# Eclectic-Sheep/sheeprl

Measured on NVIDIA H100. Metric: Dreamer-V3 train-steps/sec (S, bs16 seq64 horizon15, 64x64x3 obs), higher is better.
Workload: dtype f32

## Files before the change

include/b200rl.h:

```cpp
#ifndef B200RL_H_
#define B200RL_H_

#include <cuda_runtime_api.h>

#ifdef __cplusplus
extern "C" {
#endif

const char* b200rl_last_error(void);
int b200rl_abi_version(void);
const char* b200rl_build_arch(void);
int b200rl_device_check(void);

int b200rl_gemm_f32(const float* A, const float* B, float* C, const float* bias, int M, int N, int K, int lda, int ldb,
                    int ldc, int transA, int transB, int accumulate, cudaStream_t stream);
int b200rl_set_matmul_precision(int tf32_passes);
int b200rl_get_matmul_precision(void);
int b200rl_gemm_tc_supported(const float* A, const float* B, int M, int N, int K, int lda, int ldb, int transA,
                             int transB);
int b200rl_gemm_tc(const float* A, const float* B, float* C, const float* bias, int M, int N, int K, int lda, int ldb,
                   int ldc, int transA, int transB, int accumulate, cudaStream_t stream);
int b200rl_gemm_ln_supported(const float* A, const float* W, int M, int N, int K, int lda, int ldw, int mode);
int b200rl_gemm_ln(const float* A, const float* W, int M, int N, int K, int lda, int ldw, const float* gamma,
                   const float* beta, float eps, int act, float* pre, long long ldpre, float* out, long long ldout,
                   int mode, const float* h_prev, long long ldh, float* h_out, long long ldho, float* h_out2,
                   long long ldho2, cudaStream_t stream);
int b200rl_ln_act_fwd(const float* X, const float* gamma, const float* beta, float* Y, long long M, int C,
                      long long ldx, long long ldy, float eps, int act, cudaStream_t stream);
int b200rl_ln_act_bwd(const float* X, const float* gamma, const float* beta, const float* dY, float* dX, float* dgamma,
                      float* dbeta, long long M, int C, long long ldx, long long lddy, long long lddx, float eps,
                      int act, int accumulate, cudaStream_t stream);
int b200rl_col_sum(const float* X, float* out, long long M, int C, long long ldx, int accumulate, cudaStream_t stream);

int b200rl_obs_prep(const void* obs_nchw, int is_uint8, float* out_nhwc, long long NB, int C, int HW,
                    cudaStream_t stream);
int b200rl_transpose_batched(const float* X, float* Y, int NB, int a, int b, cudaStream_t stream);
int b200rl_transpose2d(const float* X, float* Y, int rows, int cols, long long ldx, long long ldy, cudaStream_t stream);
int b200rl_conv_down(const float* big, const float* W, float* small_, int NB, int h, int w, int Cs, int Cb,
                     cudaStream_t stream);
int b200rl_conv_up(const float* small_, const float* W, float* big, const float* bias, int NB, int h, int w, int Cs,
                   int Cb, cudaStream_t stream);
int b200rl_conv_wgrad(const float* small_, const float* big, float* dW, int NB, int h, int w, int Cs, int Cb,
                      int accumulate, cudaStream_t stream);
int b200rl_thin_down_supported(int w, int Cs, int Cb);
int b200rl_thin_up_supported(int Cs, int Cb);
int b200rl_thin_wgrad_supported(int Cs, int Cb);
int b200rl_conv_wgrad_tc_supported(int NB, int h, int w, int Cs, int Cb);
long long b200rl_conv_wgrad_tc_workspace(int NB, int h, int w, int Cs, int Cb);
int b200rl_conv_wgrad_tc(const float* small_, const float* big, float* dW, float* workspace, int NB, int h, int w,
                         int Cs, int Cb, int accumulate, cudaStream_t stream);
int b200rl_conv_tc_supported(int mode_up, int NB, int h, int w, int Cs, int Cb);
long long b200rl_conv_pack_floats(int mode_up, int Cs, int Cb);
int b200rl_conv_pack(const float* W, float* Wpacked, int mode_up, int Cs, int Cb, cudaStream_t stream);
int b200rl_conv_down_tc(const float* big, const float* Wpacked, float* small_, int NB, int h, int w, int Cs, int Cb,
                        cudaStream_t stream);
int b200rl_conv_up_tc(const float* small_, const float* Wpacked, float* big, const float* bias, int NB, int h, int w,
                      int Cs, int Cb, cudaStream_t stream);

int b200rl_gru_gate_fwd(const float* G, const float* Hin, float* Hout, long long M, int R, long long ldg,
                        long long ldhi, long long ldho, cudaStream_t stream);
int b200rl_gru_gate_bwd(const float* G, const float* Hin, const float* dH, float* dG, float* dHin, long long M, int R,
                        long long ldg, long long ldhi, long long lddh, long long lddg, long long lddhi,
                        cudaStream_t stream);
int b200rl_mask_mix(const float* prev, const float* init_row, const float* first, float* out, long long M, int C,
                    long long ldp, long long ldo, cudaStream_t stream);
int b200rl_mask_bwd(const float* dIn, const float* first, float* dPrev, float* dInit, int M, int C, long long ldi,
                    long long ldp, cudaStream_t stream);
int b200rl_cat_sample(const float* raw, const float* noise, float* onehot, float* mix_out, long long M, int groups,
                      int classes, long long ldr, long long ldn, long long ldo, long long ldm, float unimix,
                      cudaStream_t stream);
int b200rl_head_sample_supported(const float* X, const float* W, int Kin, int A, long long ldx, long long ldw);
int b200rl_head_sample(const float* X, const float* W, const float* bias, const float* noise, float* raw, float* onehot,
                       long long M, int Kin, int A, long long ldx, long long ldw, long long ldr, long long ldn,
                       long long ldo, float unimix, cudaStream_t stream);
int b200rl_cat_sample_bwd(const float* raw, const float* dz, const float* dmix, float* draw, long long M, int groups,
                          int classes, long long ldr, long long lddz, long long lddm, long long lddr, float unimix,
                          cudaStream_t stream);
int b200rl_kl_loss_grad(const float* post_mix, const float* prior_mix, float* d_post, float* d_prior, float* rows,
                        long long M, int groups, int classes, long long ldp, long long ldq, long long lddp,
                        long long lddq, float kl_dyn, float kl_rep, float free_nats, float regularizer, float scale,
                        cudaStream_t stream);
typedef struct b200rl_rssm_scan_args {
  int T, B, S, D, R, A, Dx, Dt, Dr, ld_lat, ld_wr1;
  float eps, unimix;
  const float *W_in, *lnx_g, *lnx_b, *W_g, *lng_g, *lng_b, *W_t1, *lnt_g, *lnt_b, *W_t2, *b_t2;
  const float *W_r1, *lnr_g, *lnr_b, *W_r2, *b_r2;
  const float *h0, *z0;
  const float *pe, *actions, *first, *noise;
  float* latent;
  float *z_in, *h_in, *a_in, *x_pre, *x_act, *g_pre, *g_ln, *tr_pre, *tr_act, *rp_pre, *rp_act;
  float *post_raw, *prior_raw, *post_mix, *prior_mix;
  void* workspace;
  long long workspace_bytes;
} b200rl_rssm_scan_args;
typedef struct b200rl_rssm_scan_grads {
  const float *d_latent, *d_post_mix, *d_prior_mix;
  float *d_post_raw, *d_prior_raw, *d_rp_act, *d_rp_pre, *d_tr_act, *d_tr_pre, *d_g_ln, *d_g_pre, *d_x_act, *d_x_pre;
  float* d_h0;
  const float *q_r, *q_g, *q_x;
} b200rl_rssm_scan_grads;
long long b200rl_rssm_scan_workspace_bytes(int T, int B, int S, int D, int Dx, int R, int Dr);
int b200rl_rssm_scan_fwd(const b200rl_rssm_scan_args* args, cudaStream_t stream);
int b200rl_rssm_scan_bwd(const b200rl_rssm_scan_args* args, const b200rl_rssm_scan_grads* grads, cudaStream_t stream);
int b200rl_rssm_scan_check(const b200rl_rssm_scan_args* args, int backward);
int b200rl_rssm_scan_error(const void* workspace, cudaStream_t stream);
int b200rl_rssm_scan_profile(const void* workspace, long long* out64, cudaStream_t stream);

int b200rl_mse_loss_grad(const float* pred, const float* target, float* loss_row, float* grad, long long M, int P,
                         float scale, cudaStream_t stream);
int b200rl_twohot_loss_grad(const float* logits, const float* x, const float* weight, float* loss_row, float* dlogits,
                            long long M, int nbins, long long ldl, long long ldd, float low, float high, float scale,
                            int accumulate, cudaStream_t stream);
int b200rl_bce_loss_grad(const float* logit, const float* target, float* loss_row, float* dlogit, long long M,
                         float loss_scale, float scale, cudaStream_t stream);
int b200rl_twohot_mean(const float* logits, float* out, long long M, int nbins, long long ldl, float low, float high,
                       cudaStream_t stream);
int b200rl_lambda_returns(const float* rew, const float* val, const float* cont_logit, const float* true_cont,
                          float* lam, float* discount, int H, int N, float gamma, float lmbda, cudaStream_t stream);
int b200rl_moments_update(const float* x, long long n, float* state_low_high, float* out_offset_invscale, float decay,
                          float max_, float p_low, float p_high, cudaStream_t stream);
int b200rl_actor_loss_grad(const float* raw, const float* actions, const float* lam, const float* val,
                           const float* discount, const float* moments, float* rows, float* draw, long long M,
                           const int* head_dims_host, int n_heads, float unimix, float ent_coef, float scale,
                           cudaStream_t stream);
int b200rl_sum_rows(const float* X, float* out, long long M, int C, long long ldx, float scale, cudaStream_t stream);
int b200rl_weighted_mean(const float* x, const float* w, float* out, long long n, float scale, cudaStream_t stream);

int b200rl_sumsq(const float* x, long long n, double* out, cudaStream_t stream);
int b200rl_adam_step(float* p, const float* g, float* m, float* v, const double* normsq, const int* step_dev,
                     float* norm_out, long long n, float max_norm, float lr, float b1, float b2, float eps,
                     cudaStream_t stream);
int b200rl_adam_step_wd(float* p, const float* g, float* m, float* v, const double* normsq, const int* step_dev,
                        float* norm_out, long long n, float max_norm, float lr, float b1, float b2, float eps,
                        float weight_decay, cudaStream_t stream);
int b200rl_rmsprop_step(float* p, const float* g, float* square_avg, float* momentum_buf, float* grad_avg,
                        const double* normsq, float* norm_out, long long n, float max_norm, float lr, float alpha,
                        float eps, float weight_decay, float momentum, cudaStream_t stream);
int b200rl_ema(float* target, const float* src, long long n, float tau, cudaStream_t stream);
int b200rl_fill_exponential(float* out, long long n, unsigned long long seed, unsigned int stream_id,
                            const int* counter_dev, cudaStream_t stream);
int b200rl_zero(float* x, long long n, cudaStream_t stream);
int b200rl_copy2d(const float* src, float* dst, long long M, int C, long long lds, long long ldd, cudaStream_t stream);
int b200rl_axpy(const float* x, float* y, long long n, float alpha, cudaStream_t stream);
int b200rl_affine(const float* x, float* y, long long n, float alpha, float beta, cudaStream_t stream);
int b200rl_symlog(const float* x, float* y, long long M, int C, long long ldx, long long ldy, cudaStream_t stream);
int b200rl_tanh_fwd(const float* x, float* y, long long n, cudaStream_t stream);
int b200rl_tanh_bwd(const float* y, const float* dy, float* dx, long long n, int accumulate, cudaStream_t stream);
int b200rl_increment(int* p, cudaStream_t stream);

int b200rl_replay_gather(const void* storage, const long long* idx, void* out, int n_samples, int batch, int seq_len,
                         long long row_bytes, cudaStream_t stream);
int b200rl_replay_scatter(const void* src, const long long* dst_rows, void* storage, long long n_rows,
                          long long row_bytes, cudaStream_t stream);
int b200rl_gae(const float* rewards, const float* values, const float* dones, const float* next_value, float* returns,
               float* advantages, int T, int E, float gamma, float lmbda, cudaStream_t stream);

int b200rl_bgemm(const float* A, long long sam, long long sak, long long strideA, const float* B, long long sbk,
                 long long sbn, long long strideB, float* C, long long ldc, long long strideC, const float* bias,
                 long long strideBias, const float* aux, long long ldaux, long long strideAux, float* rsum,
                 long long strideRsum, int M, int N, int K, int nets, int epilogue, int accumulate, cudaStream_t stream);
int b200rl_sac_sample_fwd(const float* head, const float* eps, const float* scale, const float* abias, float* action,
                          long long ld_action, float* logp, float* tanh_out, int B, int A, cudaStream_t stream);
int b200rl_sac_sample_bwd(const float* head, const float* eps, const float* tanh_y, const float* scale,
                          const float* dact, long long stride_net, int nets, const float* log_alpha, float* dhead, int B,
                          int A, cudaStream_t stream);
int b200rl_sac_target(const float* q_target, long long stride_net, int nets, const float* logp, const float* rewards,
                      const float* terminated, const float* log_alpha, float gamma, float* y, int B, cudaStream_t stream);
int b200rl_sac_critic_loss(const float* q, long long stride_net, int nets, const float* y, float* dq, float* loss_out,
                           int B, cudaStream_t stream);
int b200rl_sac_actor_loss(const float* q, long long stride_net, int nets, const float* logp, const float* log_alpha,
                          float target_entropy, float* dq, float* actor_loss, float* alpha_loss, float* dlog_alpha, int B,
                          cudaStream_t stream);
int b200rl_fill_normal(float* out, long long n, unsigned long long seed, unsigned int stream_id, const int* counter_dev,
                       cudaStream_t stream);

int b200rl_droq_actor_loss(const float* q, long long stride_net, int nets, const float* logp, const float* log_alpha,
                           float target_entropy, float* dq, float* actor_loss, float* alpha_loss, float* dlog_alpha,
                           int B, cudaStream_t stream);
int b200rl_dropout_mask(unsigned int* mask, long long n_words, float p, unsigned long long seed, unsigned int stream_id,
                        const int* counter_dev, cudaStream_t stream);
int b200rl_dropout_ln_relu_supported(int H);
int b200rl_dropout_ln_relu_fwd(const float* z, const unsigned int* mask, float p, const float* gamma, const float* beta,
                               long long stride_param, float eps, float* y, float* stats, int nets, int B, int H,
                               cudaStream_t stream);
int b200rl_dropout_ln_relu_bwd(const float* dy, const float* y, const float* z, const unsigned int* mask, float p,
                               const float* stats, const float* gamma, long long stride_param, float* dz, float* dgamma,
                               float* dbeta, int nets, int B, int H, cudaStream_t stream);

int b200rl_im2col(const float* x, float* col, int B, int H, int W, int C, int k, int stride, cudaStream_t stream);
int b200rl_col2im(const float* dcol, const float* act, float* dx, int B, int H, int W, int C, int k, int stride,
                  cudaStream_t stream);
int b200rl_ppo_loss(const float* head, const float* actions, const float* old_logp, const float* adv,
                    const float* values, const float* old_values, const float* returns, float* dhead, float* dvalues,
                    float* losses, int B, const int* head_dims, int n_heads, int is_continuous, int clip_vloss,
                    int normalize_adv, float clip_coef, float vf_coef, float ent_coef, cudaStream_t stream);

int b200rl_ppo_loss_masked(const float* head, const float* actions, const float* old_logp, const float* adv,
                           const float* values, const float* old_values, const float* returns, const float* mask,
                           float* dhead, float* dvalues, float* losses, int B, const int* head_dims, int n_heads,
                           int is_continuous, int clip_vloss, int normalize_adv, float clip_coef, float vf_coef,
                           float ent_coef, cudaStream_t stream);
int b200rl_a2c_loss(const float* head, const float* actions, const float* adv, const float* values, const float* returns,
                    float* dhead, float* dvalues, float* losses, int N, int seg, const int* head_dims, int n_heads,
                    int is_continuous, int normalize_adv, int reduce_sum, float vf_coef, float ent_coef,
                    cudaStream_t stream);
int b200rl_lstm_seq_fwd(const float* xw, const float* W_hh, const float* h0, const float* c0, const int* lengths,
                        float* out, float* gates, float* cs, float* hT, float* cT, int T, int B, int H,
                        cudaStream_t stream);
int b200rl_lstm_seq_bwd(const float* d_out, const float* W_hh, const float* gates, const float* cs, const float* c0,
                        const int* lengths, float* d_gates, int T, int B, int H, cudaStream_t stream);

int b200rl_onehot_linear_supported(int S, int K, int A, int N);
int b200rl_onehot_linear(const float* z, const float* act, const float* WT, float* out, long long M, int S, int K, int A,
                         int N, long long ldz, long long lda, long long ldo, cudaStream_t stream);
int b200rl_onehot_linear_ln_supported(const float* WT, const float* gamma, const float* beta, const float* out,
                                      const float* pre, int N, long long ldo, long long ldpre);
int b200rl_onehot_linear_ln(const float* z, const float* act, const float* WT, const float* gamma, const float* beta,
                            float eps, float* pre, long long ldpre, float* out, long long M, int S, int K, int A, int N,
                            long long ldz, long long lda, long long ldo, cudaStream_t stream);

int b200rl_cont_action_fwd(const float* head, const float* eps, float* action, long long lda, float* ent, long long M,
                           int A, float min_std, float max_std, float init_std, float clip, cudaStream_t stream);
int b200rl_cont_action_bwd(const float* head, const float* eps, const float* d_action, long long ldd,
                           const float* discount, float* dhead, long long M, int A, float min_std, float max_std,
                           float init_std, float clip, float ent_scale, cudaStream_t stream);
int b200rl_lambda_returns_bwd(const float* cont_logit, const float* discount, const float* moments, const float* lam,
                              const float* val, const float* ent, float* d_val, float* d_rew, float* rows, int H, int N,
                              float gamma, float lmbda, float ent_coef, float scale, cudaStream_t stream);
int b200rl_twohot_mean_bwd(const float* logits, const float* d_mean, float* d_logits, long long M, int nb, long long ldl,
                           long long ldd, float low, float high, cudaStream_t stream);

int b200rl_conv_wgrad_mn_supported(int NB, int h, int w, int Cs, int Cb);
int b200rl_conv_wgrad_mn(const float* small_, const float* big, float* G, int NB, int h, int w, int Cs, int Cb,
                         cudaStream_t stream);

int b200rl_ppo_act(const float* head, const float* noise, float* actions, float* logp, int B, const int* head_dims,
                   int n_heads, int is_continuous, int greedy, cudaStream_t stream);

#ifdef __cplusplus
}
#endif
#endif
```

sheeprl_b200/csrc/gemm_tc.cu:

```cuda
#include <cuda.h>
#include <cudaTypedefs.h>

#include <mutex>
#include <unordered_map>

#include "common.cuh"

namespace {

constexpr int BM = 128, BK = 32;
constexpr int NTHREADS = 384;
constexpr int NSPLIT_THREADS = 96;
constexpr int NCONS_WARPS = 8;
constexpr int PRODUCER_REGS = 56, CONSUMER_REGS = 224;
template <int BN> constexpr int stages_for() { return BN == 128 ? 3 : 5; }

__device__ __forceinline__ uint32_t smem_u32(const void* p) { return (uint32_t)__cvta_generic_to_shared(p); }

__device__ __forceinline__ void mbar_init(uint64_t* bar, uint32_t count) {
  asm volatile("mbarrier.init.shared::cta.b64 [%0], %1;" ::"r"(smem_u32(bar)), "r"(count) : "memory");
}
__device__ __forceinline__ void mbar_expect_tx(uint64_t* bar, uint32_t bytes) {
  asm volatile("mbarrier.arrive.expect_tx.shared::cta.b64 _, [%0], %1;" ::"r"(smem_u32(bar)), "r"(bytes) : "memory");
}
__device__ __forceinline__ void mbar_arrive(uint64_t* bar) {
  asm volatile("mbarrier.arrive.shared::cta.b64 _, [%0];" ::"r"(smem_u32(bar)) : "memory");
}
__device__ __forceinline__ bool mbar_try_wait(uint64_t* bar, uint32_t parity) {
  uint32_t ok;
  asm volatile(
      "{\n\t"
      ".reg .pred p;\n\t"
      "mbarrier.try_wait.parity.shared::cta.b64 p, [%1], %2;\n\t"
      "selp.u32 %0, 1, 0, p;\n\t"
      "}"
      : "=r"(ok)
      : "r"(smem_u32(bar)), "r"(parity)
      : "memory");
  return ok != 0;
}
__device__ __forceinline__ void mbar_wait(uint64_t* bar, uint32_t parity) {
  if (mbar_try_wait(bar, parity)) return;
  const long long t0 = clock64();
  while (!mbar_try_wait(bar, parity)) {
    if (clock64() - t0 > 2000000000LL) asm volatile("trap;");
  }
}
__device__ __forceinline__ bool elect_one() {
  uint32_t pred;
  asm volatile(
      "{\n\t"
      ".reg .pred p;\n\t"
      "elect.sync _|p, 0xffffffff;\n\t"
      "selp.u32 %0, 1, 0, p;\n\t"
      "}"
      : "=r"(pred));
  return pred != 0;
}
__device__ __forceinline__ void tma_load_2d(void* smem_dst, const CUtensorMap* map, uint64_t* bar, int c0, int c1) {
  asm volatile(
      "cp.async.bulk.tensor.2d.shared::cluster.global.mbarrier::complete_tx::bytes [%0], [%1, {%3, %4}], [%2];" ::"r"(
          smem_u32(smem_dst)),
      "l"(map), "r"(smem_u32(bar)), "r"(c0), "r"(c1)
      : "memory");
}
__device__ __forceinline__ void tma_load_4d(void* smem_dst, const CUtensorMap* map, uint64_t* bar, int c0, int c1, int c2,
                                            int c3) {
  asm volatile(
      "cp.async.bulk.tensor.4d.shared::cluster.global.mbarrier::complete_tx::bytes [%0], [%1, {%3, %4, %5, %6}], [%2];" ::"r"(
          smem_u32(smem_dst)),
      "l"(map), "r"(smem_u32(bar)), "r"(c0), "r"(c1), "r"(c2), "r"(c3)
      : "memory");
}

__device__ __forceinline__ void wgmma_tf32(float (&d)[32], const uint32_t (&a)[4], uint64_t desc_b, int scale_d) {
  asm volatile(
      "{\n\t.reg .pred p;\n\tsetp.ne.b32 p, %37, 0;\n\twgmma.mma_async.sync.aligned.m64n64k8.f32.tf32.tf32 {%0, %1, %2, %3, %4, %5, %6, %7, %8, %9, %10, %11, %12, %13, %14, %15, %16, %17, %18, %19, %20, %21, %22, %23, %24, %25, %26, %27, %28, %29, %30, %31}, {%32, %33, %34, %35}, %36, p, 1, 1;\n\t}"
      : "+f"(d[0]), "+f"(d[1]), "+f"(d[2]), "+f"(d[3]), "+f"(d[4]), "+f"(d[5]), "+f"(d[6]), "+f"(d[7]), "+f"(d[8]), "+f"(d[9]), "+f"(d[10]), "+f"(d[11]), "+f"(d[12]), "+f"(d[13]), "+f"(d[14]), "+f"(d[15]), "+f"(d[16]), "+f"(d[17]), "+f"(d[18]), "+f"(d[19]), "+f"(d[20]), "+f"(d[21]), "+f"(d[22]), "+f"(d[23]), "+f"(d[24]), "+f"(d[25]), "+f"(d[26]), "+f"(d[27]), "+f"(d[28]), "+f"(d[29]), "+f"(d[30]), "+f"(d[31])
      : "r"(a[0]), "r"(a[1]), "r"(a[2]), "r"(a[3]), "l"(desc_b), "r"(scale_d));
}
__device__ __forceinline__ void wgmma_tf32(float (&d)[64], const uint32_t (&a)[4], uint64_t desc_b, int scale_d) {
  asm volatile(
      "{\n\t.reg .pred p;\n\tsetp.ne.b32 p, %69, 0;\n\twgmma.mma_async.sync.aligned.m64n128k8.f32.tf32.tf32 {%0, %1, %2, %3, %4, %5, %6, %7, %8, %9, %10, %11, %12, %13, %14, %15, %16, %17, %18, %19, %20, %21, %22, %23, %24, %25, %26, %27, %28, %29, %30, %31, %32, %33, %34, %35, %36, %37, %38, %39, %40, %41, %42, %43, %44, %45, %46, %47, %48, %49, %50, %51, %52, %53, %54, %55, %56, %57, %58, %59, %60, %61, %62, %63}, {%64, %65, %66, %67}, %68, p, 1, 1;\n\t}"
      : "+f"(d[0]), "+f"(d[1]), "+f"(d[2]), "+f"(d[3]), "+f"(d[4]), "+f"(d[5]), "+f"(d[6]), "+f"(d[7]), "+f"(d[8]), "+f"(d[9]), "+f"(d[10]), "+f"(d[11]), "+f"(d[12]), "+f"(d[13]), "+f"(d[14]), "+f"(d[15]), "+f"(d[16]), "+f"(d[17]), "+f"(d[18]), "+f"(d[19]), "+f"(d[20]), "+f"(d[21]), "+f"(d[22]), "+f"(d[23]), "+f"(d[24]), "+f"(d[25]), "+f"(d[26]), "+f"(d[27]), "+f"(d[28]), "+f"(d[29]), "+f"(d[30]), "+f"(d[31]), "+f"(d[32]), "+f"(d[33]), "+f"(d[34]), "+f"(d[35]), "+f"(d[36]), "+f"(d[37]), "+f"(d[38]), "+f"(d[39]), "+f"(d[40]), "+f"(d[41]), "+f"(d[42]), "+f"(d[43]), "+f"(d[44]), "+f"(d[45]), "+f"(d[46]), "+f"(d[47]), "+f"(d[48]), "+f"(d[49]), "+f"(d[50]), "+f"(d[51]), "+f"(d[52]), "+f"(d[53]), "+f"(d[54]), "+f"(d[55]), "+f"(d[56]), "+f"(d[57]), "+f"(d[58]), "+f"(d[59]), "+f"(d[60]), "+f"(d[61]), "+f"(d[62]), "+f"(d[63])
      : "r"(a[0]), "r"(a[1]), "r"(a[2]), "r"(a[3]), "l"(desc_b), "r"(scale_d));
}
__device__ __forceinline__ void wgmma_fence() { asm volatile("wgmma.fence.sync.aligned;" ::: "memory"); }
__device__ __forceinline__ void wgmma_commit() { asm volatile("wgmma.commit_group.sync.aligned;" ::: "memory"); }
__device__ __forceinline__ void wgmma_wait_all() { asm volatile("wgmma.wait_group.sync.aligned 0;" ::: "memory"); }
template <int N>
__device__ __forceinline__ void fence_regs(float (&r)[N]) {
#pragma unroll
  for (int i = 0; i < N; ++i) asm volatile("" : "+f"(r[i])::"memory");
}
template <int N, int W>
__device__ __forceinline__ void fence_regs(uint32_t (&r)[N][W]) {
#pragma unroll
  for (int i = 0; i < N; ++i)
#pragma unroll
    for (int j = 0; j < W; ++j) asm volatile("" : "+r"(r[i][j])::"memory");
}

__device__ __forceinline__ uint64_t make_desc(uint32_t smem_addr) {
  uint64_t d = 0;
  d |= (uint64_t)((smem_addr & 0x3FFFF) >> 4);
  d |= (uint64_t)1 << 16;
  d |= (uint64_t)(1024 >> 4) << 32;
  d |= (uint64_t)1 << 62;
  return d;
}

__device__ __forceinline__ uint32_t kmajor_off(int r, int k) {
  return (uint32_t)(r * 128 + ((((k >> 2) ^ r) & 7) << 4) + (k & 3) * 4);
}
__device__ __forceinline__ uint32_t mnmajor_off(int r, int k) {
  return (uint32_t)((r >> 5) * 4096 + k * 128 + (((((r & 31) >> 2) ^ k) & 7) << 4) + (r & 3) * 4);
}

template <int BN>
struct Smem {
  static constexpr int STAGES = stages_for<BN>();
  float a[STAGES][BM * BK];
  float b[STAGES][BN * BK];
  float b_hi[STAGES][BN * BK];
  float b_lo[STAGES][BN * BK];
  uint64_t full[STAGES], split[STAGES], empty[STAGES];
};

constexpr int CH = 4;

constexpr int MODE_GEMM = 0, MODE_DOWN = 1, MODE_UP = 2;
constexpr int MODE_UP4 = 3;
constexpr int GROUP_M = 16;
struct TileGeo {
  int mode;
  int h, w, NB;
  int bw, bh, bn;
  int tiles_x, tiles_y;
  int chunks;
  int Cout;
  int ksplits;
  float* part;
  int mpad, ldw;
  int force_part;
  int passes;
  int a_mn, b_mn;
  int mtiles;
  int ntiles;
  int wg;
};

template <int BN, int PASSES>
__global__ void __launch_bounds__(NTHREADS, 1)
gemm_tc_kernel(const __grid_constant__ CUtensorMap mapA, const __grid_constant__ CUtensorMap mapB, float* __restrict__ C,
               const float* __restrict__ bias, int M, int N, int K, int ldc, int accumulate, const TileGeo geo) {
  constexpr int STAGES = Smem<BN>::STAGES;
  extern __shared__ __align__(1024) unsigned char smem_raw[];
  Smem<BN>& s = *reinterpret_cast<Smem<BN>*>(smem_raw + ((1024u - (smem_u32(smem_raw) & 1023u)) & 1023u));
  const int warp = threadIdx.x >> 5, lane = threadIdx.x & 31;
  const int mtiles = geo.mtiles * geo.ntiles, tstride = gridDim.y;
  auto tile_mn = [&](int id, int& tm, int& tn) {
    if (geo.ntiles == 1) { tm = id; tn = 0; return; }
    const int per = GROUP_M * geo.ntiles, grp = id / per, first = grp * GROUP_M;
    const int gsz = min(GROUP_M, geo.mtiles - first), r = id - grp * per;
    tn = r / gsz;
    tm = first + (r - tn * gsz);
  };
  int kb_base = 0, nkb = (K + BK - 1) / BK;
  if (geo.mode == MODE_GEMM && geo.ksplits > 1) {
    const int per = (nkb + geo.ksplits - 1) / geo.ksplits;
    kb_base = (int)blockIdx.z * per;
    nkb = min(per, nkb - kb_base);
  }
  const int py = (int)blockIdx.z >> 1, px = (int)blockIdx.z & 1;
  auto tile_origin = [&](int id, int& tx0, int& ty0, int& tn0) {
    tx0 = (id % geo.tiles_x) * geo.bw;
    ty0 = ((id / geo.tiles_x) % geo.tiles_y) * geo.bh;
    tn0 = (id / (geo.tiles_x * geo.tiles_y)) * geo.bn;
  };

  if (threadIdx.x == 0) {
    for (int i = 0; i < STAGES; ++i) {
      mbar_init(&s.full[i], 1);
      mbar_init(&s.split[i], NSPLIT_THREADS / 32);
      mbar_init(&s.empty[i], NCONS_WARPS);
    }
    asm volatile("fence.mbarrier_init.release.cluster;" ::: "memory");
  }
  __syncthreads();

  if (warp < 4) {
    asm volatile("setmaxnreg.dec.sync.aligned.u32 %0;" ::"n"(PRODUCER_REGS));
    if (warp == 0) {
      const bool leader = elect_one();
      int it = 0;
      for (int tile = blockIdx.y; tile < mtiles; tile += tstride) {
        int tm, tn;
        tile_mn(tile, tm, tn);
        const int m0 = tm * BM, n0 = tn * BN;
        int tx0 = 0, ty0 = 0, tn0 = 0;
        if (geo.mode != MODE_GEMM) tile_origin(tm, tx0, ty0, tn0);
        for (int kb = 0; kb < nkb; ++kb, ++it) {
          const int st = it % STAGES;
          if (it >= STAGES) mbar_wait(&s.empty[st], ((it / STAGES) - 1) & 1);
          if (leader) {
            mbar_expect_tx(&s.full[st], (uint32_t)((BM + BN) * BK * sizeof(float)));
            if (geo.mode == MODE_GEMM) {
              const int k0 = (kb_base + kb) * BK;
              if (geo.wg) {
                const int x0 = k0 % geo.w, y0 = (k0 / geo.w) % geo.h, i0 = k0 / (geo.w * geo.h);
                for (int j = 0; j < BM / 32; ++j) {
                  const int r0 = m0 + 32 * j, tap = r0 / geo.Cout, ch = r0 - tap * geo.Cout;
                  tma_load_4d(s.a[st] + j * 1024, &mapA, &s.full[st], ch, 2 * x0 - 1 + (tap & 3), 2 * y0 - 1 + (tap >> 2), i0);
                }
              } else if (!geo.a_mn) tma_load_2d(s.a[st], &mapA, &s.full[st], k0, m0);
              else
                for (int j = 0; j < BM / 32; ++j) tma_load_2d(s.a[st] + j * 1024, &mapA, &s.full[st], m0 + 32 * j, k0);
              if (!geo.b_mn) tma_load_2d(s.b[st], &mapB, &s.full[st], k0, n0);
              else
                for (int j = 0; j < BN / 32; ++j) tma_load_2d(s.b[st] + j * 1024, &mapB, &s.full[st], n0 + 32 * j, k0);
            } else {
              const int tap = kb / geo.chunks, ch = (kb - tap * geo.chunks) * BK;
              int x, y;
              if (geo.mode == MODE_DOWN)     { x = 2 * tx0 - 1 + (tap & 3); y = 2 * ty0 - 1 + (tap >> 2); }
              else if (geo.mode == MODE_UP4) { x = tx0 + (tap % 3) - 1;     y = ty0 + (tap / 3) - 1; }
              else                           { x = tx0 + px - (tap & 1);    y = ty0 + py - (tap >> 1); }
              tma_load_4d(s.a[st], &mapA, &s.full[st], ch, x, y, tn0);
              tma_load_2d(s.b[st], &mapB, &s.full[st], kb * BK, n0 + (geo.mode == MODE_UP ? (int)blockIdx.z * geo.Cout : 0));
            }
          }
          __syncwarp();
        }
      }
    } else {
      const int t = threadIdx.x - 32;
      int ntl = 0;
      for (int tile = blockIdx.y; tile < mtiles; tile += tstride) ++ntl;
      const int total_kb = ntl * nkb;
      const bool b_mn = geo.b_mn != 0;
      for (int kb = 0; kb < total_kb; ++kb) {
        const int st = kb % STAGES;
        mbar_wait(&s.full[st], (kb / STAGES) & 1);
        const char* raw = reinterpret_cast<const char*>(s.b[st]);
        char* bh = reinterpret_cast<char*>(s.b_hi[st]);
        char* bl = reinterpret_cast<char*>(s.b_lo[st]);
#pragma unroll 4
        for (int w = t; w < BN * BK / 4; w += NSPLIT_THREADS) {
          int n, kc;
          float4 v;
          if (!b_mn) {
            n = w >> 3; kc = w & 7;
            v = *reinterpret_cast<const float4*>(raw + kmajor_off(n, 4 * kc));
          } else {
            n = w % BN; kc = w / BN;
            v.x = *reinterpret_cast<const float*>(raw + mnmajor_off(n, 4 * kc));
            v.y = *reinterpret_cast<const float*>(raw + mnmajor_off(n, 4 * kc + 1));
            v.z = *reinterpret_cast<const float*>(raw + mnmajor_off(n, 4 * kc + 2));
            v.w = *reinterpret_cast<const float*>(raw + mnmajor_off(n, 4 * kc + 3));
          }
          float4 h;
          h.x = __uint_as_float(__float_as_uint(v.x) & 0xffffe000u);
          h.y = __uint_as_float(__float_as_uint(v.y) & 0xffffe000u);
          h.z = __uint_as_float(__float_as_uint(v.z) & 0xffffe000u);
          h.w = __uint_as_float(__float_as_uint(v.w) & 0xffffe000u);
          const uint32_t o = kmajor_off(n, 4 * kc);
          *reinterpret_cast<float4*>(bh + o) = h;
          if (PASSES == 3) *reinterpret_cast<float4*>(bl + o) = make_float4(v.x - h.x, v.y - h.y, v.z - h.z, v.w - h.w);
        }
        asm volatile("fence.proxy.async.shared::cta;" ::: "memory");
        __syncwarp();
        if (lane == 0) mbar_arrive(&s.split[st]);
      }
    }
  } else {
    asm volatile("setmaxnreg.inc.sync.aligned.u32 %0;" ::"n"(CONSUMER_REGS));
    constexpr int NACC = BN / 2;
    const int cw = (warp >> 2) - 1, wq = warp & 3, g = lane >> 2, tq = lane & 3;
    const int r0 = cw * 64 + wq * 16 + g;
    const bool a_mn_tile = geo.a_mn != 0;
    const uint64_t dbh_base = make_desc(smem_u32(s.b_hi[0])), dbl_base = make_desc(smem_u32(s.b_lo[0]));
    constexpr uint64_t STAGE_STEP = (uint64_t)(BN * BK * sizeof(float)) >> 4;
    int it = 0;
    for (int tile = blockIdx.y; tile < mtiles; tile += tstride) {
      int tm, tn;
      tile_mn(tile, tm, tn);
      const int m0 = tm * BM, n0 = tn * BN;
      int tx0 = 0, ty0 = 0, tn0 = 0;
      if (geo.mode != MODE_GEMM) tile_origin(tm, tx0, ty0, tn0);
      float acc[NACC], cacc[NACC];
#pragma unroll
      for (int j = 0; j < NACC; ++j) { acc[j] = 0.f; cacc[j] = 0.f; }
      for (int kb = 0; kb < nkb; ++kb, ++it) {
        const int st = it % STAGES;
        const uint32_t ph = (it / STAGES) & 1;
        mbar_wait(&s.full[st], ph);
        mbar_wait(&s.split[st], ph);
        const char* araw = reinterpret_cast<const char*>(s.a[st]);
        uint32_t ahi[4][4], alo[4][4];
#pragma unroll
        for (int ks = 0; ks < 4; ++ks)
#pragma unroll
          for (int e = 0; e < 4; ++e) {
            const int r = r0 + 8 * (e & 1), k = 8 * ks + tq + 4 * (e >> 1);
            const uint32_t x = *reinterpret_cast<const uint32_t*>(araw + (a_mn_tile ? mnmajor_off(r, k) : kmajor_off(r, k)));
            ahi[ks][e] = x & 0xffffe000u;
            if (PASSES == 3) alo[ks][e] = __float_as_uint(__uint_as_float(x) - __uint_as_float(x & 0xffffe000u));
          }
        const bool chunk_start = (kb % CH) == 0;
        const uint64_t dbh0 = dbh_base + (uint64_t)st * STAGE_STEP, dbl0 = dbl_base + (uint64_t)st * STAGE_STEP;
        fence_regs(cacc);
        fence_regs(ahi);
        if (PASSES == 3) fence_regs(alo);
        wgmma_fence();
#pragma unroll
        for (int ks = 0; ks < 4; ++ks) {
          const uint64_t ob = (uint64_t)ks * 2;
          const int keep = !(chunk_start && ks == 0);
          if (PASSES == 3) {
            wgmma_tf32(cacc, ahi[ks], dbl0 + ob, keep);
            wgmma_tf32(cacc, alo[ks], dbh0 + ob, 1);
            wgmma_tf32(cacc, ahi[ks], dbh0 + ob, 1);
          } else {
            wgmma_tf32(cacc, ahi[ks], dbh0 + ob, keep);
          }
        }
        wgmma_commit();
        wgmma_wait_all();
        fence_regs(cacc);
        fence_regs(ahi);
        if (PASSES == 3) fence_regs(alo);
        __syncwarp();
        if (lane == 0) mbar_arrive(&s.empty[st]);
        if ((kb % CH) == CH - 1 || kb == nkb - 1) {
#pragma unroll
          for (int j = 0; j < NACC; ++j) acc[j] += cacc[j];
        }
      }
#pragma unroll
      for (int hh = 0; hh < 2; ++hh) {
        const int r = r0 + 8 * hh;
        const int row = m0 + r;
        bool row_ok = row < M;
        size_t row_off = (size_t)row * ldc;
        int wi = 0, hi = 0, ni = 0;
        if (geo.mode != MODE_GEMM) {
          wi = r % geo.bw; hi = (r / geo.bw) % geo.bh; ni = r / (geo.bw * geo.bh);
          const int n = tn0 + ni, y = ty0 + hi, x = tx0 + wi;
          row_ok = n < geo.NB;
          if (geo.mode == MODE_DOWN) row_off = (((size_t)n * geo.h + y) * geo.w + x) * (size_t)ldc;
          else row_off = (((size_t)n * (2 * geo.h) + (2 * y + py)) * (2 * geo.w) + (2 * x + px)) * (size_t)ldc;
        }
        if (geo.mode == MODE_UP4) {
          if (!row_ok) continue;
          const size_t n = (size_t)(tn0 + ni);
          const int y = ty0 + hi, x = tx0 + wi;
#pragma unroll
          for (int j = 0; j < NACC / 4; ++j) {
            const int c = 8 * j + 2 * tq, p = c >> 5, ch = c & 31;
            float* dst = C + ((n * (2 * geo.h) + (2 * y + (p >> 1))) * (2 * geo.w) + (2 * x + (p & 1))) * (size_t)32 + ch;
            float2 o = make_float2(acc[4 * j + 2 * hh], acc[4 * j + 2 * hh + 1]);
            if (bias) { o.x += bias[ch]; o.y += bias[ch + 1]; }
            *reinterpret_cast<float2*>(dst) = o;
          }
          continue;
        }
        if (geo.mode == MODE_GEMM && (geo.ksplits > 1 || geo.force_part)) {
          float* prow = geo.part + ((size_t)blockIdx.z * geo.mpad + (size_t)row) * geo.ldw + n0;
#pragma unroll
          for (int j = 0; j < NACC / 4; ++j)
            *reinterpret_cast<float2*>(prow + 8 * j + 2 * tq) = make_float2(acc[4 * j + 2 * hh], acc[4 * j + 2 * hh + 1]);
          continue;
        }
        if (!row_ok) continue;
        float* crow = C + row_off;
#pragma unroll
        for (int j = 0; j < NACC / 4; ++j) {
          const int cb = n0 + 8 * j + 2 * tq;
          float v0 = acc[4 * j + 2 * hh], v1 = acc[4 * j + 2 * hh + 1];
          if (cb + 1 < N && ((reinterpret_cast<uintptr_t>(crow + cb) & 7) == 0)) {
            if (bias) { v0 += bias[cb]; v1 += bias[cb + 1]; }
            if (accumulate) { const float2 q = *reinterpret_cast<const float2*>(crow + cb); v0 += q.x; v1 += q.y; }
            *reinterpret_cast<float2*>(crow + cb) = make_float2(v0, v1);
          } else {
            if (cb < N) crow[cb] = v0 + (bias ? bias[cb] : 0.f) + (accumulate ? crow[cb] : 0.f);
            if (cb + 1 < N) crow[cb + 1] = v1 + (bias ? bias[cb + 1] : 0.f) + (accumulate ? crow[cb + 1] : 0.f);
          }
        }
      }
    }
  }
}

struct MapKey {
  const void* ptr; int rows, cols, ld, box_rows;
  bool operator==(const MapKey& o) const { return ptr == o.ptr && rows == o.rows && cols == o.cols && ld == o.ld && box_rows == o.box_rows; }
};
struct MapHash {
  size_t operator()(const MapKey& k) const {
    size_t h = std::hash<const void*>()(k.ptr);
    h ^= std::hash<long long>()(((long long)k.rows << 32) ^ k.cols) + 0x9e3779b97f4a7c15ull + (h << 6) + (h >> 2);
    h ^= std::hash<long long>()(((long long)k.ld << 8) ^ k.box_rows) + 0x9e3779b97f4a7c15ull + (h << 6) + (h >> 2);
    return h;
  }
};
std::unordered_map<MapKey, CUtensorMap, MapHash> g_maps;
std::mutex g_maps_mu;

typedef CUresult (*EncodeTiledFn)(CUtensorMap*, CUtensorMapDataType, cuuint32_t, void*, const cuuint64_t*, const cuuint64_t*,
                                  const cuuint32_t*, const cuuint32_t*, CUtensorMapInterleave, CUtensorMapSwizzle,
                                  CUtensorMapL2promotion, CUtensorMapFloatOOBfill);
EncodeTiledFn encode_tiled() {
  static EncodeTiledFn fn = nullptr;
  if (!fn) {
    void* p = nullptr;
    cudaDriverEntryPointQueryResult q;
    if (cudaGetDriverEntryPoint("cuTensorMapEncodeTiled", &p, cudaEnableDefault, &q) == cudaSuccess &&
        q == cudaDriverEntryPointSuccess)
      fn = reinterpret_cast<EncodeTiledFn>(p);
  }
  return fn;
}

int get_map(const float* ptr, int rows, int cols, int ld, int box_rows, CUtensorMap* out) {
  MapKey key{ptr, rows, cols, ld, box_rows};
  std::lock_guard<std::mutex> lk(g_maps_mu);
  auto it = g_maps.find(key);
  if (it != g_maps.end()) { *out = it->second; return B200RL_OK; }
  CUtensorMap m;
  cuuint64_t dims[2] = {(cuuint64_t)cols, (cuuint64_t)rows};
  cuuint64_t strides[1] = {(cuuint64_t)ld * sizeof(float)};
  cuuint32_t box[2] = {(cuuint32_t)BK, (cuuint32_t)box_rows};
  cuuint32_t estr[2] = {1, 1};
  EncodeTiledFn enc = encode_tiled();
  if (!enc) { b200rl_set_error("cuTensorMapEncodeTiled is not available from this driver"); return B200RL_ERR_CUDA; }
  CUresult r = enc(&m, CU_TENSOR_MAP_DATA_TYPE_FLOAT32, 2, const_cast<float*>(ptr), dims, strides, box,
                                      estr, CU_TENSOR_MAP_INTERLEAVE_NONE,
                                      CU_TENSOR_MAP_SWIZZLE_128B,
                                      CU_TENSOR_MAP_L2_PROMOTION_L2_256B, CU_TENSOR_MAP_FLOAT_OOB_FILL_NONE);
  if (r != CUDA_SUCCESS) {
    b200rl_set_error("cuTensorMapEncodeTiled failed (%d) for [%d x %d] ld %d", (int)r, rows, cols, ld);
    return B200RL_ERR_CUDA;
  }
  if (g_maps.size() > 4096) g_maps.clear();
  g_maps.emplace(key, m);
  *out = m;
  return B200RL_OK;
}

struct Map4Key {
  const void* ptr; int C, W, H, N, bw, bh, bn, es;
  bool operator==(const Map4Key& o) const {
    return ptr == o.ptr && C == o.C && W == o.W && H == o.H && N == o.N && bw == o.bw && bh == o.bh && bn == o.bn && es == o.es;
  }
};
struct Map4Hash {
  size_t operator()(const Map4Key& k) const {
    size_t h = std::hash<const void*>()(k.ptr);
    const long long v[4] = {((long long)k.C << 32) ^ k.W, ((long long)k.H << 32) ^ k.N, ((long long)k.bw << 32) ^ k.bh,
                            ((long long)k.bn << 32) ^ k.es};
    for (long long x : v) h ^= std::hash<long long>()(x) + 0x9e3779b97f4a7c15ull + (h << 6) + (h >> 2);
    return h;
  }
};
std::unordered_map<Map4Key, CUtensorMap, Map4Hash> g_maps4;

int get_map4(const float* ptr, int C, int W, int H, int N, int bw, int bh, int bn, int es, CUtensorMap* out) {
  Map4Key key{ptr, C, W, H, N, bw, bh, bn, es};
  std::lock_guard<std::mutex> lk(g_maps_mu);
  auto it = g_maps4.find(key);
  if (it != g_maps4.end()) { *out = it->second; return B200RL_OK; }
  CUtensorMap m;
  cuuint64_t dims[4] = {(cuuint64_t)C, (cuuint64_t)W, (cuuint64_t)H, (cuuint64_t)N};
  cuuint64_t strides[3] = {(cuuint64_t)C * 4, (cuuint64_t)C * W * 4, (cuuint64_t)C * W * H * 4};
  cuuint32_t box[4] = {(cuuint32_t)BK, (cuuint32_t)((bw - 1) * es + 1), (cuuint32_t)((bh - 1) * es + 1), (cuuint32_t)bn};
  cuuint32_t estr[4] = {1, (cuuint32_t)es, (cuuint32_t)es, 1};
  EncodeTiledFn enc = encode_tiled();
  if (!enc) { b200rl_set_error("cuTensorMapEncodeTiled is not available from this driver"); return B200RL_ERR_CUDA; }
  CUresult r = enc(&m, CU_TENSOR_MAP_DATA_TYPE_FLOAT32, 4, const_cast<float*>(ptr), dims, strides, box,
                                      estr, CU_TENSOR_MAP_INTERLEAVE_NONE,
                                      CU_TENSOR_MAP_SWIZZLE_128B,
                                      CU_TENSOR_MAP_L2_PROMOTION_L2_256B, CU_TENSOR_MAP_FLOAT_OOB_FILL_NONE);
  if (r != CUDA_SUCCESS) {
    b200rl_set_error("cuTensorMapEncodeTiled(4D) failed (%d) for image [%d,%d,%d,%d]", (int)r, N, H, W, C);
    return B200RL_ERR_CUDA;
  }
  if (g_maps4.size() > 1024) g_maps4.clear();
  g_maps4.emplace(key, m);
  *out = m;
  return B200RL_OK;
}

bool conv_tile(int h, int w, int NB, int* bw, int* bh, int* bn) {
  if (w <= 0 || h <= 0 || (w & (w - 1)) || (h & (h - 1))) return false;
  *bw = w < 128 ? w : 128;
  int rest = 128 / *bw;
  *bh = h < rest ? h : rest;
  *bn = rest / *bh;
  return (w % *bw == 0) && (h % *bh == 0) && (*bw * *bh * *bn == 128) && (NB % *bn == 0);
}

static unsigned persistent_grid_y(int tiles, unsigned gz) {
  const long long total = (long long)tiles * gz;
  if (total <= 2LL * kNumSMs) return (unsigned)tiles;
  unsigned gy = kNumSMs / gz;
  if (gy < 1) gy = 1;
  return gy < (unsigned)tiles ? gy : (unsigned)tiles;
}

__global__ void conv_pack_down_kernel(const float* __restrict__ W, float* __restrict__ P, int Cs, int Cb) {
  const long long idx = (long long)blockIdx.x * blockDim.x + threadIdx.x;
  if (idx >= (long long)Cs * Cb * 16) return;
  const int cb = (int)(idx % Cb);
  const int tap = (int)((idx / Cb) % 16);
  const int cs = (int)(idx / ((long long)Cb * 16));
  P[idx] = W[((long long)cs * Cb + cb) * 16 + tap];
}
__global__ void conv_pack_up_kernel(const float* __restrict__ W, float* __restrict__ P, int Cs, int Cb) {
  const long long idx = (long long)blockIdx.x * blockDim.x + threadIdx.x;
  if (idx >= (long long)Cs * Cb * 16) return;
  const int cs = (int)(idx % Cs);
  const int t = (int)((idx / Cs) % 4);
  const int cb = (int)((idx / ((long long)Cs * 4)) % Cb);
  const int par = (int)(idx / ((long long)Cs * 4 * Cb));
  const int py = par >> 1, px = par & 1;
  const int ky = (1 - py) + 2 * (t >> 1), kx = (1 - px) + 2 * (t & 1);
  P[idx] = W[((long long)cs * Cb + cb) * 16 + ky * 4 + kx];
}

__global__ void conv_pack_up4_kernel(const float* __restrict__ W, float* __restrict__ P, int Cs, int Cb) {
  const long long idx = (long long)blockIdx.x * blockDim.x + threadIdx.x;
  if (idx >= 36LL * Cs * Cb) return;
  const int cs = (int)(idx % Cs);
  const int shift = (int)((idx / Cs) % 9);
  const int cb = (int)((idx / (9LL * Cs)) % Cb);
  const int par = (int)(idx / (9LL * Cs * Cb));
  const int py = par >> 1, px = par & 1, dy = shift / 3 - 1, dx = shift % 3 - 1;
  const int j = py - dy, i = px - dx;
  float v = 0.f;
  if (j >= 0 && j <= 1 && i >= 0 && i <= 1) v = W[((long long)cs * Cb + cb) * 16 + ((1 - py) + 2 * j) * 4 + (1 - px) + 2 * i];
  P[idx] = v;
}
static bool conv_up_merged(int Cb) { return Cb == 32; }

int g_passes = 3;

struct SplitWs {
  float* part = nullptr;
  size_t floats = 0;
};
SplitWs g_split[16];
std::mutex g_split_mu;

int split_workspace(size_t need_floats, cudaStream_t st, float** part) {
  int dev = 0;
  RL_CUDA(cudaGetDevice(&dev));
  RL_CHECK_ARG(dev < 16, "split-K workspace: device index out of range");
  std::lock_guard<std::mutex> lk(g_split_mu);
  SplitWs& w = g_split[dev];
  if (need_floats > w.floats) {
    cudaStreamCaptureStatus cs = cudaStreamCaptureStatusNone;
    RL_CUDA(cudaStreamIsCapturing(st, &cs));
    if (cs != cudaStreamCaptureStatusNone) {
      b200rl_set_error("split-K workspace must grow during stream capture: run the step once eagerly first");
      return B200RL_ERR_CUDA;
    }
    RL_CUDA(cudaDeviceSynchronize());
    if (w.part) RL_CUDA(cudaFree(w.part));
    const size_t n = need_floats + need_floats / 2 > (size_t)16 << 20 ? need_floats + need_floats / 2 : (size_t)16 << 20;
    RL_CUDA(cudaMalloc(&w.part, n * sizeof(float)));
    w.floats = n;
  }
  *part = w.part;
  return B200RL_OK;
}

__global__ void __launch_bounds__(256)
splitk_reduce_kernel(const float* __restrict__ part, float* __restrict__ C, const float* __restrict__ bias, int M, int N,
                     int ldc, int ks, int mpad, int ldw, int accumulate) {
  const int n4 = (N + 3) >> 2;
  const long long idx = (long long)blockIdx.x * blockDim.x + threadIdx.x;
  if (idx >= (long long)M * n4) return;
  const int m = (int)(idx / n4), n = (int)(idx - (long long)m * n4) * 4;
  const float* p = part + (size_t)m * ldw + n;
  float4 acc = make_float4(0.f, 0.f, 0.f, 0.f);
#pragma unroll 4
  for (int z = 0; z < ks; ++z) {
    const float4 v = __ldcg(reinterpret_cast<const float4*>(p + (size_t)z * mpad * ldw));
    acc.x += v.x; acc.y += v.y; acc.z += v.z; acc.w += v.w;
  }
  float* c = C + (size_t)m * ldc + n;
  const float o[4] = {acc.x, acc.y, acc.z, acc.w};
  if (n + 4 <= N && ((reinterpret_cast<uintptr_t>(c) & 15) == 0)) {
    float4 r = acc;
    if (bias) { r.x += bias[n]; r.y += bias[n + 1]; r.z += bias[n + 2]; r.w += bias[n + 3]; }
    if (accumulate) { const float4 q = *reinterpret_cast<const float4*>(c); r.x += q.x; r.y += q.y; r.z += q.z; r.w += q.w; }
    *reinterpret_cast<float4*>(c) = r;
  } else {
    for (int j = 0; j < 4 && n + j < N; ++j) {
      float r = o[j];
      if (bias) r += bias[n + j];
      if (accumulate) r += c[j];
      c[j] = r;
    }
  }
}

#define LAUNCH_GEMM_TC(BN_, PASSES_, grid_, st_, ...)                                                                \
  do {                                                                                                               \
    const size_t smem__ = sizeof(Smem<BN_>) + 1024;                                                                  \
    RL_CUDA(cudaFuncSetAttribute(gemm_tc_kernel<BN_, PASSES_>, cudaFuncAttributeMaxDynamicSharedMemorySize, (int)smem__)); \
    gemm_tc_kernel<BN_, PASSES_><<<grid_, NTHREADS, smem__, st_>>>(__VA_ARGS__);                                      \
  } while (0)
#define DISPATCH_GEMM_TC(BN_val, passes_val, grid_, st_, ...)                                  \
  do {                                                                                          \
    if ((BN_val) == 64) {                                                                       \
      if ((passes_val) == 3) LAUNCH_GEMM_TC(64, 3, grid_, st_, __VA_ARGS__);                    \
      else LAUNCH_GEMM_TC(64, 1, grid_, st_, __VA_ARGS__);                                      \
    } else {                                                                                    \
      if ((passes_val) == 3) LAUNCH_GEMM_TC(128, 3, grid_, st_, __VA_ARGS__);                   \
      else LAUNCH_GEMM_TC(128, 1, grid_, st_, __VA_ARGS__);                                     \
    }                                                                                           \
  } while (0)

int launch_conv(int mode, const float* img, const float* Wp, float* out, const float* bias, int NB, int h, int w, int Cin,
                int Cout, cudaStream_t st) {
  TileGeo g = {};
  g.mode = mode; g.h = h; g.w = w; g.NB = NB; g.chunks = Cin / BK; g.Cout = Cout; g.ksplits = 1;
  g.passes = g_passes;
  RL_CHECK_ARG(conv_tile(h, w, NB, &g.bw, &g.bh, &g.bn), "image grid not tileable by 128 pixels");
  g.tiles_x = w / g.bw; g.tiles_y = h / g.bh;
  if (mode == MODE_UP && conv_up_merged(Cout)) mode = g.mode = MODE_UP4;
  const int taps = mode == MODE_DOWN ? 16 : (mode == MODE_UP4 ? 9 : 4);
  const int K = taps * Cin;
  CUtensorMap ma, mb;
  if (mode == MODE_DOWN) { if (int rc = get_map4(img, Cin, 2 * w, 2 * h, NB, g.bw, g.bh, g.bn, 2, &ma)) return rc; }
  else                   { if (int rc = get_map4(img, Cin, w, h, NB, g.bw, g.bh, g.bn, 1, &ma)) return rc; }
  const int BN = (mode == MODE_UP4) ? 128 : ((Cout <= 64) ? 64 : 128);
  const int brows = (mode == MODE_UP || mode == MODE_UP4) ? 4 * Cout : Cout;
  if (int rc = get_map(Wp, brows, K, K, BN, &mb)) return rc;
  const int mtiles = g.tiles_x * g.tiles_y * (NB / g.bn);
  g.mtiles = mtiles;
  g.ntiles = (mode == MODE_UP4) ? 1 : (Cout + BN - 1) / BN;
  dim3 grid(1, 1, mode == MODE_UP ? 4 : 1);
  grid.y = persistent_grid_y(mtiles * g.ntiles, grid.z);
  const int M = NB * h * w;
  DISPATCH_GEMM_TC(BN, g.passes, grid, st, ma, mb, out, bias, M, Cout, K, Cout, 0, g);
  RL_CHECK_LAUNCH();
  return B200RL_OK;
}

}

extern "C" int b200rl_set_matmul_precision(int tf32_passes) {
  RL_CHECK_ARG(tf32_passes == 1 || tf32_passes == 3, "tf32_passes must be 3 (fp32-accurate 3xTF32) or 1 (single TF32 pass)");
  g_passes = tf32_passes;
  return B200RL_OK;
}
extern "C" int b200rl_get_matmul_precision(void) { return g_passes; }

extern "C" long long b200rl_conv_pack_floats(int mode_up, int Cs, int Cb) {
  return (mode_up && conv_up_merged(Cb) ? 36LL : 16LL) * Cs * Cb;
}
extern "C" int b200rl_conv_tc_supported(int mode_up, int NB, int h, int w, int Cs, int Cb) {
  int bw, bh, bn;
  if (!conv_tile(h, w, NB, &bw, &bh, &bn)) return 0;
  const int Cin = mode_up ? Cs : Cb, Cout = mode_up ? Cb : Cs;
  if (Cin % BK != 0 || Cout < 16 || Cout % 4 != 0) return 0;
  return 1;
}
extern "C" int b200rl_conv_pack(const float* W, float* Wpacked, int mode_up, int Cs, int Cb, cudaStream_t st) {
  RL_CHECK_ARG(W && Wpacked, "null pointer");
  const long long n = (long long)Cs * Cb * 16;
  if (mode_up && conv_up_merged(Cb)) conv_pack_up4_kernel<<<ceil_div(36LL * Cs * Cb, 256), 256, 0, st>>>(W, Wpacked, Cs, Cb);
  else if (mode_up) conv_pack_up_kernel<<<ceil_div(n, 256), 256, 0, st>>>(W, Wpacked, Cs, Cb);
  else conv_pack_down_kernel<<<ceil_div(n, 256), 256, 0, st>>>(W, Wpacked, Cs, Cb);
  RL_CHECK_LAUNCH();
  return B200RL_OK;
}
extern "C" int b200rl_conv_down_tc(const float* big, const float* Wpacked, float* small_, int NB, int h, int w, int Cs,
                                   int Cb, cudaStream_t st) {
  RL_CHECK_ARG(big && Wpacked && small_, "null pointer");
  RL_CHECK_ARG(b200rl_conv_tc_supported(0, NB, h, w, Cs, Cb), "shape not eligible for the tensor-core conv path");
  return launch_conv(MODE_DOWN, big, Wpacked, small_, nullptr, NB, h, w, Cb, Cs, st);
}
extern "C" int b200rl_conv_up_tc(const float* small_, const float* Wpacked, float* big, const float* bias, int NB, int h,
                                 int w, int Cs, int Cb, cudaStream_t st) {
  RL_CHECK_ARG(big && Wpacked && small_, "null pointer");
  RL_CHECK_ARG(b200rl_conv_tc_supported(1, NB, h, w, Cs, Cb), "shape not eligible for the tensor-core conv path");
  return launch_conv(MODE_UP, small_, Wpacked, big, bias, NB, h, w, Cs, Cb, st);
}

extern "C" int b200rl_gemm_tc_supported(const float* A, const float* B, int M, int N, int K, int lda, int ldb,
                                        int transA, int transB) {
  (void)transA; (void)transB;
  if (M < 32 || N < 48 || K < 32) return 0;
  if ((lda & 3) || (ldb & 3)) return 0;
  if ((reinterpret_cast<uintptr_t>(A) & 15) || (reinterpret_cast<uintptr_t>(B) & 15)) return 0;
  return 1;
}

namespace {
struct FusedTail { float* part; int ks, mpad, ldw; };

int gemm_tc_impl(const float* A, const float* B, float* C, const float* bias, int M, int N, int K, int lda,
                 int ldb, int ldc, int transA, int transB, int accumulate, cudaStream_t st, FusedTail* fused) {
  RL_CHECK_ARG(A && B && (C || fused), "null pointer");
  RL_CHECK_ARG(b200rl_gemm_tc_supported(A, B, M, N, K, lda, ldb, transA, transB), "shape not eligible for the tensor-core path");
  const int BN = (N <= 64) ? 64 : 128;
  CUtensorMap ma, mb;
  if (!transA) { if (int rc = get_map(A, M, K, lda, BM, &ma)) return rc; }
  else         { if (int rc = get_map(A, K, M, lda, 32, &ma)) return rc; }
  if (transB)  { if (int rc = get_map(B, N, K, ldb, BN, &mb)) return rc; }
  else         { if (int rc = get_map(B, K, N, ldb, 32, &mb)) return rc; }
  dim3 grid((N + BN - 1) / BN, (M + BM - 1) / BM);
  TileGeo g = {};
  g.mode = MODE_GEMM;
  g.a_mn = transA ? 1 : 0;
  g.b_mn = transB ? 0 : 1;
  g.ksplits = 1;
  g.passes = g_passes;
  const int tiles = grid.x * grid.y, nkb = (K + BK - 1) / BK;
  if (tiles < 2 * kNumSMs && nkb >= 8) {
    int best = 1;
    float best_t = 1e30f;
    const int max_sp = nkb / 4 < 32 ? nkb / 4 : 32;
    for (int sp = 1; sp <= (max_sp < 1 ? 1 : max_sp); ++sp) {
      const int per = (nkb + sp - 1) / sp, real = (nkb + per - 1) / per;
      const int waves = (tiles * real + kNumSMs - 1) / kNumSMs;
      const float t = waves * (per * 0.8f + 4.0f) + (real > 1 ? 3.0f + 0.3f * real : 0.0f);
      if (t < best_t - 1e-3f) { best_t = t; best = real; }
    }
    g.ksplits = best;
  }
  if (g.ksplits > 1 || fused) {
    grid.z = g.ksplits;
    g.mpad = (int)grid.y * BM;
    g.ldw = (int)grid.x * BN;
    if (int rc = split_workspace((size_t)g.ksplits * g.mpad * g.ldw, st, &g.part)) return rc;
    if (fused) { g.force_part = 1; *fused = FusedTail{g.part, g.ksplits, g.mpad, g.ldw}; }
  }
  g.mtiles = (int)grid.y;
  g.ntiles = (int)grid.x;
  grid.x = 1;
  grid.y = persistent_grid_y(g.mtiles * g.ntiles, grid.z);
  DISPATCH_GEMM_TC(BN, g.passes, grid, st, ma, mb, C, bias, M, N, K, ldc, accumulate, g);
  RL_CHECK_LAUNCH();
  if (g.ksplits > 1 && !fused) {
    splitk_reduce_kernel<<<ceil_div((long long)M * ((N + 3) / 4), 256), 256, 0, st>>>(g.part, C, bias, M, N, ldc, g.ksplits, g.mpad,
                                                                                      g.ldw, accumulate);
    RL_CHECK_LAUNCH();
  }
  return B200RL_OK;
}

template <int NV>
__global__ void __launch_bounds__(256)
splitk_ln_kernel(const float* __restrict__ part, int ks, int mpad, int ldw, int M, int N, const float* __restrict__ gamma,
                 const float* __restrict__ beta, float eps, int act, float* __restrict__ pre, long long ldpre,
                 float* __restrict__ ln_out, long long ldln, int mode, const float* __restrict__ h_prev, long long ldh,
                 float* __restrict__ h_out, long long ldho, float* __restrict__ h_out2, long long ldho2) {
  const int lane = threadIdx.x & 31;
  const long long row = ((long long)blockIdx.x * blockDim.x + threadIdx.x) >> 5;
  if (row >= M) return;
  const int n4 = N >> 2;
  float4 v[NV];
#pragma unroll
  for (int i = 0; i < NV; ++i) v[i] = make_float4(0.f, 0.f, 0.f, 0.f);
#pragma unroll 4
  for (int z = 0; z < ks; ++z) {
    const float4* p = reinterpret_cast<const float4*>(part + ((size_t)z * mpad + row) * ldw);
#pragma unroll
    for (int i = 0; i < NV; ++i) {
      const int c = lane + 32 * i;
      if (c < n4) { const float4 t = __ldcg(p + c); v[i].x += t.x; v[i].y += t.y; v[i].z += t.z; v[i].w += t.w; }
    }
  }
  float s = 0.f;
#pragma unroll
  for (int i = 0; i < NV; ++i) {
    const int c = lane + 32 * i;
    if (c < n4) {
      if (pre) reinterpret_cast<float4*>(pre + row * ldpre)[c] = v[i];
      s += (v[i].x + v[i].y) + (v[i].z + v[i].w);
    }
  }
  const float mu = warp_sum(s) / (float)N;
  float q = 0.f;
#pragma unroll
  for (int i = 0; i < NV; ++i) {
    const int c = lane + 32 * i;
    if (c < n4) {
      const float dx = v[i].x - mu, dy = v[i].y - mu, dz = v[i].z - mu, dw = v[i].w - mu;
      q += (dx * dx + dy * dy) + (dz * dz + dw * dw);
    }
  }
  const float rstd = rsqrtf(warp_sum(q) / (float)N + eps);
#pragma unroll
  for (int i = 0; i < NV; ++i) {
    const int c = lane + 32 * i;
    if (c < n4) {
      const float4 g = reinterpret_cast<const float4*>(gamma)[c], b = reinterpret_cast<const float4*>(beta)[c];
      v[i].x = (v[i].x - mu) * rstd * g.x + b.x; v[i].y = (v[i].y - mu) * rstd * g.y + b.y;
      v[i].z = (v[i].z - mu) * rstd * g.z + b.z; v[i].w = (v[i].w - mu) * rstd * g.w + b.w;
      if (mode == 0 && act == 1) {
        v[i].x = v[i].x / (1.f + expf(-v[i].x)); v[i].y = v[i].y / (1.f + expf(-v[i].y));
        v[i].z = v[i].z / (1.f + expf(-v[i].z)); v[i].w = v[i].w / (1.f + expf(-v[i].w));
      }
      if (ln_out) reinterpret_cast<float4*>(ln_out + row * ldln)[c] = v[i];
    }
  }
  if (mode == 1) {
    constexpr int NR = NV / 3;
#pragma unroll
    for (int i = 0; i < NR; ++i) {
      const int c = lane + 32 * i;
      const float4 hp = reinterpret_cast<const float4*>(h_prev + row * ldh)[c];
      const float4 gr = v[i], gc = v[i + NR], gu = v[i + 2 * NR];
      float4 h;
      auto gate = [](float r_, float c_, float u_, float hprev) {
        const float r = 1.f / (1.f + expf(-r_));
        const float cand = tanhf(r * c_);
        const float u = 1.f / (1.f + expf(-(u_ - 1.f)));
        return u * cand + (1.f - u) * hprev;
      };
      h.x = gate(gr.x, gc.x, gu.x, hp.x); h.y = gate(gr.y, gc.y, gu.y, hp.y);
      h.z = gate(gr.z, gc.z, gu.z, hp.z); h.w = gate(gr.w, gc.w, gu.w, hp.w);
      reinterpret_cast<float4*>(h_out + row * ldho)[c] = h;
      if (h_out2) reinterpret_cast<float4*>(h_out2 + row * ldho2)[c] = h;
    }
  }
}
}

extern "C" int b200rl_gemm_tc(const float* A, const float* B, float* C, const float* bias, int M, int N, int K, int lda,
                              int ldb, int ldc, int transA, int transB, int accumulate, cudaStream_t st) {
  return gemm_tc_impl(A, B, C, bias, M, N, K, lda, ldb, ldc, transA, transB, accumulate, st, nullptr);
}

extern "C" int b200rl_gemm_ln_supported(const float* A, const float* B, int M, int N, int K, int lda, int ldb, int mode) {
  if (!b200rl_gemm_tc_supported(A, B, M, N, K, lda, ldb, 0, 1)) return 0;
  if (N % 4 || N > 1536) return 0;
  if (mode == 1 && (N % 384 != 0)) return 0;
  return 1;
}

extern "C" int b200rl_gemm_ln(const float* A, const float* W, int M, int N, int K, int lda, int ldw_, const float* gamma,
                              const float* beta, float eps, int act, float* pre, long long ldpre, float* out, long long ldout,
                              int mode, const float* h_prev, long long ldh, float* h_out, long long ldho, float* h_out2,
                              long long ldho2, cudaStream_t st) {
  RL_CHECK_ARG(A && W && gamma && beta, "null pointer");
  RL_CHECK_ARG(b200rl_gemm_ln_supported(A, W, M, N, K, lda, ldw_, mode), "shape not eligible for the fused product + LayerNorm");
  RL_CHECK_ARG(mode == 0 ? out != nullptr : (h_prev && h_out), "missing output");
  RL_CHECK_ARG(((reinterpret_cast<uintptr_t>(gamma) | reinterpret_cast<uintptr_t>(beta) | reinterpret_cast<uintptr_t>(pre) |
                 reinterpret_cast<uintptr_t>(out) | reinterpret_cast<uintptr_t>(h_prev) | reinterpret_cast<uintptr_t>(h_out) |
                 reinterpret_cast<uintptr_t>(h_out2)) & 15) == 0 &&
                   ((ldpre | ldout | ldh | ldho | ldho2) & 3) == 0,
               "fused product + LayerNorm needs 16-byte aligned rows");
  FusedTail ft;
  if (int rc = gemm_tc_impl(A, W, nullptr, nullptr, M, N, K, lda, ldw_, N, 0, 1, 0, st, &ft)) return rc;
  const int blocks = ceil_div((long long)M * 32, 256);
#define LAUNCH_SPLITK_LN(NV_)                                                                                              \
  splitk_ln_kernel<NV_><<<blocks, 256, 0, st>>>(ft.part, ft.ks, ft.mpad, ft.ldw, M, N, gamma, beta, eps, act, pre, ldpre, out, \
                                                ldout, mode, h_prev, ldh, h_out, ldho, h_out2, ldho2)
  if (mode == 1) {
    if (N == 384) LAUNCH_SPLITK_LN(3); else if (N == 768) LAUNCH_SPLITK_LN(6); else if (N == 1152) LAUNCH_SPLITK_LN(9);
    else LAUNCH_SPLITK_LN(12);
  } else if (N <= 128) LAUNCH_SPLITK_LN(1);
  else if (N <= 256) LAUNCH_SPLITK_LN(2);
  else if (N <= 512) LAUNCH_SPLITK_LN(4);
  else if (N <= 1024) LAUNCH_SPLITK_LN(8);
  else LAUNCH_SPLITK_LN(12);
#undef LAUNCH_SPLITK_LN
  RL_CHECK_LAUNCH();
  return B200RL_OK;
}

extern "C" int b200rl_conv_wgrad_mn_supported(int NB, int h, int w, int Cs, int Cb) {
  if (w <= 0 || h <= 0 || (w & (w - 1)) || (h & (h - 1))) return 0;
  const long long P = (long long)NB * h * w;
  if (Cb % 32 || Cs < 48 || Cs % 4 || P % 32 || P < 1024 || P > 2000000000LL) return 0;
  const int bw = w < 32 ? w : 32, bh = (32 / bw) < h ? (32 / bw) : h, bn = 32 / (bw * bh);
  return (bw * bh * bn == 32) && (NB % bn == 0);
}

extern "C" int b200rl_conv_wgrad_mn(const float* small_, const float* big, float* G, int NB, int h, int w, int Cs, int Cb,
                                    cudaStream_t st) {
  RL_CHECK_ARG(small_ && big && G, "null pointer");
  RL_CHECK_ARG(b200rl_conv_wgrad_mn_supported(NB, h, w, Cs, Cb), "shape not eligible for the in-place wgrad path");
  const int P = NB * h * w, M = 16 * Cb, N = Cs;
  TileGeo g = {};
  g.mode = MODE_GEMM; g.a_mn = 1; g.b_mn = 1; g.wg = 1; g.passes = g_passes;
  g.h = h; g.w = w; g.NB = NB; g.Cout = Cb;
  g.bw = w < 32 ? w : 32; g.bh = (32 / g.bw) < h ? (32 / g.bw) : h; g.bn = 32 / (g.bw * g.bh);
  CUtensorMap ma, mb;
  if (int rc = get_map4(big, Cb, 2 * w, 2 * h, NB, g.bw, g.bh, g.bn, 2, &ma)) return rc;
  if (int rc = get_map(small_, P, Cs, Cs, 32, &mb)) return rc;
  const int BN = (N <= 64) ? 64 : 128;
  dim3 grid((N + BN - 1) / BN, M / BM);
  const int tiles = grid.x * grid.y, nkb = P / BK;
  int sp = (2 * kNumSMs + tiles - 1) / tiles;
  if (sp > nkb / 8) sp = nkb / 8;
  if (sp < 1) sp = 1;
  const int per = (nkb + sp - 1) / sp;
  g.ksplits = (nkb + per - 1) / per;
  grid.z = g.ksplits;
  g.mtiles = (int)grid.y;
  g.ntiles = (int)grid.x;
  if (g.ksplits > 1) {
    g.mpad = (int)grid.y * BM;
    g.ldw = (int)grid.x * BN;
    if (int rc = split_workspace((size_t)g.ksplits * g.mpad * g.ldw, st, &g.part)) return rc;
  }
  grid.x = 1;
  grid.y = (unsigned)(g.mtiles * g.ntiles);
  DISPATCH_GEMM_TC(BN, g.passes, grid, st, ma, mb, G, nullptr, M, N, P, N, 0, g);
  RL_CHECK_LAUNCH();
  if (g.ksplits > 1) {
    splitk_reduce_kernel<<<ceil_div((long long)M * ((N + 3) / 4), 256), 256, 0, st>>>(g.part, G, nullptr, M, N, N, g.ksplits, g.mpad,
                                                                                      g.ldw, 0);
    RL_CHECK_LAUNCH();
  }
  return B200RL_OK;
}
```

sheeprl_b200/lib.py:

```python
from __future__ import annotations

import ctypes
import os
import re
from typing import Optional, Sequence

import torch

_HERE = os.path.dirname(os.path.abspath(__file__))
LIB_PATH = os.path.join(_HERE, "libb200rl.so")
HEADER_PATH = os.path.join(os.path.dirname(_HERE), "include", "b200rl.h")

_lib = None


class B200RLError(RuntimeError):
    pass


_SCALARS = {"int": ctypes.c_int, "long long": ctypes.c_longlong, "unsigned int": ctypes.c_uint,
            "unsigned long long": ctypes.c_ulonglong, "float": ctypes.c_float}


def _decl(text: str, where: Optional[str] = None, result: bool = False):
    m = re.fullmatch(r"\s*(.+?)\s*\b(\w+)\s*", text, re.S)
    if m is None:
        raise B200RLError(f"{where}: cannot parse the declaration {text.strip()!r}")
    words = m.group(1).replace("*", " * ").split()
    base = " ".join(w for w in words if w not in ("const", "*"))
    if "*" in words or base == "cudaStream_t":
        return m.group(2), ctypes.c_char_p if result and base == "char" else ctypes.c_void_p
    if base not in _SCALARS:
        raise B200RLError(f"{where or m.group(2)}: C type {m.group(1)!r} has no ctypes binding")
    return m.group(2), _SCALARS[base]


def parse_header(text: str):
    text = re.sub(r"/\*.*?\*/|^\s*#[^\n]*", " ", text, flags=re.S | re.M)
    structs, typedef = {}, r"typedef\s+struct\s+\w+\s*\{(.*?)\}\s*(\w+)\s*;"
    for body, name in re.findall(typedef, text, re.S):
        structs[name] = []
        for stmt in filter(str.strip, body.split(";")):
            first, *more = stmt.split(",")
            base = re.match(r"\s*(.*?)[\s*]*\w+\s*$", first, re.S).group(1)
            structs[name] += [_decl(d, name) for d in [first] + [base + " " + d for d in more]]
    functions = {}
    for stmt in re.sub(typedef, " ", text, flags=re.S).split(";"):
        stmt = re.split(r"[{}]", stmt)[-1].strip()
        if not stmt:
            continue
        m = re.fullmatch(r"(.+?)\((.*)\)", stmt, re.S)
        if m is None:
            raise B200RLError(f"cannot parse the declaration {stmt!r}")
        name, restype = _decl(m.group(1), result=True)
        params = m.group(2).strip()
        functions[name] = (restype, [] if params in ("", "void") else [_decl(p, name)[1] for p in params.split(",")])
    return functions, structs


with open(HEADER_PATH) as _f:
    _FUNCTIONS, _STRUCTS = parse_header(_f.read())


def _bind(fn, restype, argtypes):
    fn.restype, fn.argtypes, n = restype, argtypes, len(argtypes)

    def call(*args):
        if len(args) != n:
            raise TypeError(f"{fn.__name__} takes {n} arguments ({len(args)} given)")
        return fn(*args)

    call.__name__, call.restype, call.argtypes = fn.__name__, restype, argtypes
    return call


def load_library(path: str = LIB_PATH) -> ctypes.CDLL:
    global _lib
    if _lib is None:
        if not os.path.exists(path):
            raise B200RLError(f"{path} not found: build it with `python -m sheeprl_b200.build` (nvcc, sm_90a). "
                              "The B200 engine has no CPU / PyTorch fallback.")
        lib = ctypes.CDLL(path)
        for name, (restype, argtypes) in _FUNCTIONS.items():
            setattr(lib, name, _bind(getattr(lib, name), restype, argtypes))
        _lib = lib
    return _lib


def declared_symbols() -> Sequence[str]:
    return sorted(_FUNCTIONS)


def _p(t: Optional[torch.Tensor]):
    return None if t is None else t.data_ptr()


def _ld(t: Optional[torch.Tensor]) -> int:
    if t is None:
        return 0
    if t.dim() == 1:
        assert t.numel() <= 1 or t.stride(0) == 1, "1-D views must be contiguous"
        return max(t.numel(), 1)
    assert t.dim() == 2, f"expected a 2-D view, got {tuple(t.shape)}"
    assert t.shape[1] == 1 or t.stride(1) == 1, f"inner stride must be 1, got {t.stride()}"
    return t.stride(0) if t.shape[0] > 1 else max(t.stride(0), t.shape[1])


def _f32(*ts):
    for t in ts:
        if t is not None:
            assert t.dtype == torch.float32 and t.is_cuda, (t.dtype, t.device)


def _struct(name: str, typedef: str, exclude=()):
    fields = _STRUCTS[typedef]
    pointers = tuple(n for n, t in fields if t is ctypes.c_void_p and n not in exclude)
    return type(name, (ctypes.Structure,), {"_fields_": fields, "POINTERS": pointers})


RssmScanArgs = _struct("RssmScanArgs", "b200rl_rssm_scan_args", exclude=("workspace",))
RssmScanGrads = _struct("RssmScanGrads", "b200rl_rssm_scan_grads")


class CudaOps:
    name = "cuda"

    def __init__(self, device="cuda"):
        if not torch.cuda.is_available():
            raise B200RLError("no CUDA device visible: the B200 engine has no CPU fallback")
        self.lib = load_library()
        self.device = torch.device(device)
        if self.device.index is not None:
            torch.cuda.set_device(self.device)
        if self.lib.b200rl_device_check() != 0:
            raise B200RLError(self.lib.b200rl_last_error().decode())
        self.launches = 0
        self.use_tc = os.environ.get("B200RL_DISABLE_TC", "0") != "1"
        self._pack_bufs = {}
        self._scratch_bufs = {}

    def _st(self):
        return torch.cuda.current_stream().cuda_stream

    def _ck(self, rc: int, launches: int = 1):
        self.launches += launches
        if rc != 0:
            raise B200RLError(self.lib.b200rl_last_error().decode())

    def set_matmul_precision(self, precision: str) -> None:
        p = str(precision).lower()
        if p not in ("highest", "high", "medium"):
            raise ValueError(f"float32_matmul_precision must be highest / high / medium, got {precision}")
        self._ck(self.lib.b200rl_set_matmul_precision(3 if p == "highest" else 1), 0)

    def matmul_precision(self) -> str:
        return "highest" if self.lib.b200rl_get_matmul_precision() == 3 else "high"

    def gemm(self, A, B, C, transA: bool, transB: bool, bias=None, accumulate: bool = False):
        _f32(A, B, C, bias)
        M, N = C.shape
        K = A.shape[0] if transA else A.shape[1]
        assert (A.shape[1] if transA else A.shape[0]) == M, (A.shape, C.shape, transA)
        assert (B.shape[0] if transB else B.shape[1]) == N and (B.shape[1] if transB else B.shape[0]) == K, \
            (A.shape, B.shape, C.shape, transA, transB)
        self._ck(self.lib.b200rl_gemm_f32(_p(A), _p(B), _p(C), _p(bias), M, N, K, _ld(A), _ld(B), _ld(C), int(transA),
                                          int(transB), int(accumulate), self._st()))

    def gemm_ln_supported(self, A, W, mode: int = 0) -> bool:
        M, K = A.shape
        return self.use_tc and bool(self.lib.b200rl_gemm_ln_supported(_p(A), _p(W), M, W.shape[0], K, _ld(A), _ld(W),
                                                                     mode))

    def gemm_ln_act(self, A, W, gamma, beta, eps: float, act: int, out, pre=None):
        _f32(A, W, gamma, beta, out, pre)
        M, K = A.shape
        N = W.shape[0]
        assert W.shape[1] == K and out.shape == (M, N)
        self._ck(self.lib.b200rl_gemm_ln(_p(A), _p(W), M, N, K, _ld(A), _ld(W), _p(gamma), _p(beta), eps, act, _p(pre),
                                         _ld(pre), _p(out), _ld(out), 0, None, 0, None, 0, None, 0, self._st()), 2)

    def gemm_ln_gru(self, A, W, gamma, beta, eps: float, h_prev, h_out, h_out2=None, g_pre=None, g_ln=None):
        _f32(A, W, gamma, beta, h_prev, h_out, h_out2, g_pre, g_ln)
        M, K = A.shape
        N = W.shape[0]
        assert W.shape[1] == K and h_prev.shape == (M, N // 3) and h_out.shape == (M, N // 3)
        self._ck(self.lib.b200rl_gemm_ln(_p(A), _p(W), M, N, K, _ld(A), _ld(W), _p(gamma), _p(beta), eps, 0, _p(g_pre),
                                         _ld(g_pre), _p(g_ln), _ld(g_ln), 1, _p(h_prev), _ld(h_prev), _p(h_out),
                                         _ld(h_out), _p(h_out2), _ld(h_out2), self._st()), 2)

    def _scratch(self, slot: str, numel: int) -> torch.Tensor:
        buf = self._scratch_bufs.get(slot)
        if buf is None or buf.numel() < numel:
            buf = torch.empty(numel, dtype=torch.float32, device=self.device)
            self._scratch_bufs[slot] = buf
        return buf

    def col_sum(self, X, out, accumulate: bool = False):
        _f32(X, out)
        self._ck(self.lib.b200rl_col_sum(_p(X), _p(out), X.shape[0], X.shape[1], _ld(X), int(accumulate), self._st()))

    def ln_act_fwd(self, X, gamma, beta, eps: float, act: int, Y):
        _f32(X, gamma, beta, Y)
        self._ck(self.lib.b200rl_ln_act_fwd(_p(X), _p(gamma), _p(beta), _p(Y), X.shape[0], X.shape[1], _ld(X), _ld(Y),
                                            eps, act, self._st()))

    def ln_act_bwd(self, X, gamma, beta, eps: float, act: int, dY, dX, dgamma, dbeta, accumulate: bool = False):
        _f32(X, gamma, beta, dY, dX, dgamma, dbeta)
        self._ck(self.lib.b200rl_ln_act_bwd(_p(X), _p(gamma), _p(beta), _p(dY), _p(dX), _p(dgamma), _p(dbeta),
                                            X.shape[0], X.shape[1], _ld(X), _ld(dY), _ld(dX), eps, act,
                                            int(accumulate), self._st()))

    def obs_prep(self, obs, out):
        assert obs.is_cuda and obs.is_contiguous() and out.is_contiguous()
        assert obs.dtype in (torch.uint8, torch.float32), obs.dtype
        NB, C, H, W = obs.shape
        self._ck(self.lib.b200rl_obs_prep(_p(obs), int(obs.dtype == torch.uint8), _p(out), NB, C, H * W, self._st()))

    def transpose_batched(self, X, Y):
        _f32(X, Y)
        assert X.is_contiguous() and Y.is_contiguous()
        NB, a, b = X.shape
        self._ck(self.lib.b200rl_transpose_batched(_p(X), _p(Y), NB, a, b, self._st()))

    def conv_down(self, big, W, small):
        _f32(big, W, small)
        assert big.is_contiguous() and small.is_contiguous() and W.is_contiguous()
        NB, h, w, Cs = small.shape
        Cb = big.shape[-1]
        assert tuple(big.shape) == (NB, 2 * h, 2 * w, Cb) and tuple(W.shape) == (Cs, Cb, 4, 4)
        if self.use_tc and self.lib.b200rl_conv_tc_supported(0, NB, h, w, Cs, Cb):
            Wp = self._packed(W, 0, Cs, Cb)
            self._ck(self.lib.b200rl_conv_down_tc(_p(big), _p(Wp), _p(small), NB, h, w, Cs, Cb, self._st()))
            return
        self._ck(self.lib.b200rl_conv_down(_p(big), _p(W), _p(small), NB, h, w, Cs, Cb, self._st()))

    def _packed(self, W, mode_up: int, Cs: int, Cb: int):
        key = (W.data_ptr(), mode_up)
        buf = self._pack_bufs.get(key)
        need = self.lib.b200rl_conv_pack_floats(mode_up, Cs, Cb)
        if buf is None or buf.numel() != need:
            buf = torch.empty(need, dtype=torch.float32, device=W.device)
            self._pack_bufs[key] = buf
        self._ck(self.lib.b200rl_conv_pack(_p(W), _p(buf), mode_up, Cs, Cb, self._st()))
        return buf

    def conv_up(self, small, W, big, bias=None):
        _f32(big, W, small, bias)
        assert big.is_contiguous() and small.is_contiguous() and W.is_contiguous()
        NB, h, w, Cs = small.shape
        Cb = big.shape[-1]
        assert tuple(big.shape) == (NB, 2 * h, 2 * w, Cb) and tuple(W.shape) == (Cs, Cb, 4, 4)
        if self.use_tc and self.lib.b200rl_conv_tc_supported(1, NB, h, w, Cs, Cb):
            Wp = self._packed(W, 1, Cs, Cb)
            self._ck(self.lib.b200rl_conv_up_tc(_p(small), _p(Wp), _p(big), _p(bias), NB, h, w, Cs, Cb, self._st()))
            return
        self._ck(self.lib.b200rl_conv_up(_p(small), _p(W), _p(big), _p(bias), NB, h, w, Cs, Cb, self._st()))

    def conv_wgrad(self, small, big, dW, accumulate: bool = False):
        _f32(big, dW, small)
        assert big.is_contiguous() and small.is_contiguous() and dW.is_contiguous()
        NB, h, w, Cs = small.shape
        Cb = big.shape[-1]
        assert tuple(big.shape) == (NB, 2 * h, 2 * w, Cb) and tuple(dW.shape) == (Cs, Cb, 4, 4)
        if self.use_tc and self.lib.b200rl_conv_wgrad_tc_supported(NB, h, w, Cs, Cb):
            ws = self._scratch("wgrad", self.lib.b200rl_conv_wgrad_tc_workspace(NB, h, w, Cs, Cb))
            self._ck(self.lib.b200rl_conv_wgrad_tc(_p(small), _p(big), _p(dW), _p(ws), NB, h, w, Cs, Cb,
                                                   int(accumulate), self._st()))
            return
        self._ck(self.lib.b200rl_conv_wgrad(_p(small), _p(big), _p(dW), NB, h, w, Cs, Cb, int(accumulate), self._st()))

    def gru_gate_fwd(self, G, Hin, Hout):
        _f32(G, Hin, Hout)
        M, R = Hin.shape
        self._ck(self.lib.b200rl_gru_gate_fwd(_p(G), _p(Hin), _p(Hout), M, R, _ld(G), _ld(Hin), _ld(Hout), self._st()))

    def gru_gate_bwd(self, G, Hin, dH, dG, dHin):
        _f32(G, Hin, dH, dG, dHin)
        M, R = Hin.shape
        self._ck(self.lib.b200rl_gru_gate_bwd(_p(G), _p(Hin), _p(dH), _p(dG), _p(dHin), M, R, _ld(G), _ld(Hin), _ld(dH),
                                              _ld(dG), _ld(dHin), self._st()))

    def mask_mix(self, prev, init, first, out):
        _f32(prev, init, first, out)
        M, C = out.shape
        self._ck(self.lib.b200rl_mask_mix(_p(prev), _p(init), _p(first), _p(out), M, C, _ld(prev), _ld(out), self._st()))

    def mask_rows(self, X, first, out):
        self.mask_mix(X, None, first, out)

    def mask_bwd(self, dIn, first, dPrev, dInit):
        _f32(dIn, first, dPrev, dInit)
        M, C = dIn.shape
        self._ck(self.lib.b200rl_mask_bwd(_p(dIn), _p(first), _p(dPrev), _p(dInit), M, C, _ld(dIn), _ld(dPrev),
                                          self._st()))

    def cat_sample(self, raw, noise, unimix: float, groups: int, classes: int, onehot, mix_out=None):
        _f32(raw, noise, onehot, mix_out)
        M = raw.shape[0]
        if noise is not None and noise.dim() != 2:
            noise = noise.reshape(M, -1)
        self._ck(self.lib.b200rl_cat_sample(_p(raw), _p(noise), _p(onehot), _p(mix_out), M, groups, classes, _ld(raw),
                                            _ld(noise), _ld(onehot), _ld(mix_out), unimix, self._st()))

    def head_sample_supported(self, X, W) -> bool:
        return bool(self.lib.b200rl_head_sample_supported(_p(X), _p(W), X.shape[1], W.shape[0], _ld(X), _ld(W)))

    def head_sample(self, X, W, bias, noise, unimix: float, raw, onehot):
        _f32(X, W, bias, noise, raw, onehot)
        M, Kin = X.shape
        A = W.shape[0]
        assert raw.shape == (M, A) and onehot.shape == (M, A) and W.shape[1] == Kin
        self._ck(self.lib.b200rl_head_sample(_p(X), _p(W), _p(bias), _p(noise), _p(raw), _p(onehot), M, Kin, A, _ld(X),
                                             _ld(W), _ld(raw), _ld(noise), _ld(onehot), unimix, self._st()))

    def cat_sample_bwd(self, raw, dz, dmix, unimix: float, groups: int, classes: int, draw):
        _f32(raw, dz, dmix, draw)
        self._ck(self.lib.b200rl_cat_sample_bwd(_p(raw), _p(dz), _p(dmix), _p(draw), raw.shape[0], groups, classes,
                                                _ld(raw), _ld(dz), _ld(dmix), _ld(draw), unimix, self._st()))

    def kl_loss_grad(self, post_mix, prior_mix, groups, classes, kl_dyn, kl_rep, free_nats, regularizer, scale,
                     d_post, d_prior, rows):
        _f32(post_mix, prior_mix, d_post, d_prior, rows)
        assert rows.is_contiguous() and rows.shape[1] == 4
        self._ck(self.lib.b200rl_kl_loss_grad(_p(post_mix), _p(prior_mix), _p(d_post), _p(d_prior), _p(rows),
                                              post_mix.shape[0], groups, classes, _ld(post_mix), _ld(prior_mix),
                                              _ld(d_post), _ld(d_prior), kl_dyn, kl_rep, free_nats, regularizer, scale,
                                              self._st()))

    def mse_loss_grad(self, pred, target, scale: float, loss_row, grad):
        _f32(pred, target, loss_row, grad)
        assert pred.is_contiguous() and target.is_contiguous() and grad.is_contiguous()
        M, P = pred.shape
        self._ck(self.lib.b200rl_mse_loss_grad(_p(pred), _p(target), _p(loss_row), _p(grad), M, P, scale, self._st()))

    def twohot_loss_grad(self, logits, x, weight, scale, low, high, loss_row, dlogits, accumulate: bool = False):
        _f32(logits, x, weight, loss_row, dlogits)
        M, nb = logits.shape
        assert x.numel() == M and x.is_contiguous()
        self._ck(self.lib.b200rl_twohot_loss_grad(_p(logits), _p(x), _p(weight), _p(loss_row), _p(dlogits), M, nb,
                                                  _ld(logits), _ld(dlogits), low, high, scale, int(accumulate),
                                                  self._st()))

    def bce_loss_grad(self, logit, target, loss_scale, scale, loss_row, dlogit):
        _f32(logit, target, loss_row, dlogit)
        assert logit.is_contiguous() and target.is_contiguous() and dlogit.is_contiguous()
        self._ck(self.lib.b200rl_bce_loss_grad(_p(logit), _p(target), _p(loss_row), _p(dlogit), logit.numel(),
                                               loss_scale, scale, self._st()))

    def twohot_mean(self, logits, low, high, out):
        _f32(logits, out)
        self._ck(self.lib.b200rl_twohot_mean(_p(logits), _p(out), logits.shape[0], logits.shape[1], _ld(logits), low,
                                             high, self._st()))

    def lambda_returns(self, rew, val, cont_logit, true_cont, gamma, lmbda, lam, discount):
        _f32(rew, val, cont_logit, true_cont, lam, discount)
        for t in (rew, val, cont_logit, lam, discount):
            assert t.is_contiguous()
        H, N = lam.shape
        self._ck(self.lib.b200rl_lambda_returns(_p(rew), _p(val), _p(cont_logit), _p(true_cont), _p(lam), _p(discount),
                                                H, N, gamma, lmbda, self._st()))

    def moments_update(self, x, state, decay, max_, p_low, p_high, out):
        _f32(x, state, out)
        assert x.is_contiguous()
        self._ck(self.lib.b200rl_moments_update(_p(x), x.numel(), _p(state), _p(out), decay, max_, p_low, p_high,
                                                self._st()))

    def actor_loss_grad(self, raw, actions, lam, val, discount, moments, head_dims, unimix, ent_coef, scale, rows,
                        draw):
        _f32(raw, actions, lam, val, discount, moments, rows, draw)
        for t in (raw, actions, draw):
            assert t.is_contiguous()
        hd = (ctypes.c_int * len(head_dims))(*[int(x) for x in head_dims])
        self._ck(self.lib.b200rl_actor_loss_grad(_p(raw), _p(actions), _p(lam), _p(val), _p(discount), _p(moments),
                                                 _p(rows), _p(draw), raw.shape[0], hd, len(head_dims), unimix, ent_coef,
                                                 scale, self._st()))

    def sum_rows(self, X, out, scale: float):
        _f32(X, out)
        self._ck(self.lib.b200rl_sum_rows(_p(X), _p(out), X.shape[0], X.shape[1], _ld(X), scale, self._st()))

    def weighted_mean(self, x, w, scale: float, out):
        _f32(x, w, out)
        self._ck(self.lib.b200rl_weighted_mean(_p(x), _p(w), _p(out), x.numel(), scale, self._st()))

    def sumsq(self, x, out):
        assert out.dtype == torch.float64 and x.is_contiguous()
        self._ck(self.lib.b200rl_sumsq(_p(x), x.numel(), _p(out), self._st()))

    def adam_step(self, p, g, m, v, normsq, max_norm, lr, b1, b2, eps, step_t, norm_out, weight_decay=0.0):
        _f32(p, g, m, v, norm_out)
        assert step_t.dtype == torch.int32 and normsq.dtype == torch.float64
        self._ck(self.lib.b200rl_adam_step_wd(_p(p), _p(g), _p(m), _p(v), _p(normsq), _p(step_t), _p(norm_out),
                                              p.numel(), max_norm, lr, b1, b2, eps, weight_decay, self._st()))

    def rmsprop_step(self, p, g, square_avg, momentum_buf, grad_avg, normsq, max_norm, lr, alpha, eps, weight_decay,
                     momentum, norm_out):
        _f32(p, g, square_avg, momentum_buf, grad_avg, norm_out)
        assert normsq.dtype == torch.float64
        for t in (g, square_avg, momentum_buf, grad_avg):
            assert t is None or t.numel() == p.numel()
        self._ck(self.lib.b200rl_rmsprop_step(_p(p), _p(g), _p(square_avg), _p(momentum_buf), _p(grad_avg), _p(normsq),
                                              _p(norm_out), p.numel(), max_norm, lr, alpha, eps, weight_decay, momentum,
                                              self._st()))

    def ema(self, target, src, tau: float):
        _f32(target, src)
        self._ck(self.lib.b200rl_ema(_p(target), _p(src), target.numel(), tau, self._st()))

    def fill_exponential(self, out, seed: int, stream_id: int, counter=None):
        _f32(out)
        assert out.is_contiguous()
        self._ck(self.lib.b200rl_fill_exponential(_p(out), out.numel(), seed, stream_id, _p(counter), self._st()))

    def increment(self, step_t):
        self._ck(self.lib.b200rl_increment(_p(step_t), self._st()))

    def zero(self, x):
        assert x.is_contiguous()
        if x.dtype == torch.float32:
            self._ck(self.lib.b200rl_zero(_p(x), x.numel(), self._st()))
        else:
            x.zero_()

    def copy(self, src, dst):
        _f32(src, dst)
        if src.dim() == 1:
            src, dst = src.view(1, -1), dst.view(1, -1)
        M, C = src.shape
        self._ck(self.lib.b200rl_copy2d(_p(src), _p(dst), M, C, _ld(src), _ld(dst), self._st()))

    def axpy(self, x, y, alpha: float = 1.0):
        _f32(x, y)
        assert x.is_contiguous() and y.is_contiguous()
        self._ck(self.lib.b200rl_axpy(_p(x), _p(y), x.numel(), alpha, self._st()))

    def affine(self, x, out, alpha: float, beta: float):
        _f32(x, out)
        assert x.is_contiguous() and out.is_contiguous()
        self._ck(self.lib.b200rl_affine(_p(x), _p(out), x.numel(), alpha, beta, self._st()))

    def symlog(self, x, y):
        _f32(x, y)
        M, C = x.shape
        assert tuple(y.shape) == (M, C)
        self._ck(self.lib.b200rl_symlog(_p(x), _p(y), M, C, _ld(x), _ld(y), self._st()))

    def tanh_fwd(self, x, y):
        _f32(x, y)
        self._ck(self.lib.b200rl_tanh_fwd(_p(x), _p(y), x.numel(), self._st()))

    def tanh_bwd(self, y, dy, dx, accumulate: bool = False):
        _f32(y, dy, dx)
        self._ck(self.lib.b200rl_tanh_bwd(_p(y), _p(dy), _p(dx), y.numel(), int(accumulate), self._st()))

    def rssm_scan_workspace(self, T: int, B: int, S: int, D: int, Dx: int, R: int, Dr: int) -> torch.Tensor:
        n = self.lib.b200rl_rssm_scan_workspace_bytes(T, B, S, D, Dx, R, Dr)
        return torch.zeros((n + 3) // 4, dtype=torch.int32, device=self.device)

    @staticmethod
    def _scan_dims(dims: dict) -> RssmScanArgs:
        return RssmScanArgs(**{k: int(dims[k]) for k, t in RssmScanArgs._fields_ if t is ctypes.c_int})

    def _scan_args(self, dims: dict, eps: float, unimix: float, tensors: dict, workspace: torch.Tensor):
        a = self._scan_dims(dims)
        a.eps, a.unimix = float(eps), float(unimix)
        for name in RssmScanArgs.POINTERS:
            t = tensors[name]
            assert t.is_cuda and t.dtype == torch.float32, name
            setattr(a, name, t.data_ptr())
        a.workspace, a.workspace_bytes = workspace.data_ptr(), workspace.numel() * workspace.element_size()
        return a

    def rssm_scan_fwd(self, dims: dict, eps: float, unimix: float, tensors: dict, workspace: torch.Tensor):
        a = self._scan_args(dims, eps, unimix, tensors, workspace)
        self._ck(self.lib.b200rl_rssm_scan_fwd(ctypes.byref(a), self._st()))

    def rssm_scan_supported(self, dims: dict, backward: bool) -> bool:
        return self.lib.b200rl_rssm_scan_check(ctypes.byref(self._scan_dims(dims)), int(backward)) == 0

    def rssm_scan_bwd(self, dims: dict, eps: float, unimix: float, tensors: dict, grads: dict,
                      workspace: torch.Tensor):
        a = self._scan_args(dims, eps, unimix, tensors, workspace)
        q = RssmScanGrads()
        for name in RssmScanGrads.POINTERS:
            t = grads[name]
            assert t.is_cuda and t.dtype == torch.float32 and t.is_contiguous(), name
            setattr(q, name, t.data_ptr())
        self._ck(self.lib.b200rl_rssm_scan_bwd(ctypes.byref(a), ctypes.byref(q), self._st()))

    def rssm_scan_error(self, workspace: torch.Tensor) -> int:
        return self.lib.b200rl_rssm_scan_error(_p(workspace), self._st())

    def rssm_scan_profile(self, workspace: torch.Tensor):
        out = (ctypes.c_longlong * 64)()
        self._ck(self.lib.b200rl_rssm_scan_profile(_p(workspace), out, self._st()), 0)
        return [list(out[:32]), list(out[32:])]

    def replay_gather(self, storage, idx, out, n_samples: int, batch: int, seq_len: int):
        assert storage.is_contiguous() and out.is_contiguous() and idx.dtype == torch.int64 and idx.is_contiguous()
        row_bytes = storage[0].numel() * storage.element_size()
        self._ck(self.lib.b200rl_replay_gather(_p(storage), _p(idx), _p(out), n_samples, batch, seq_len, row_bytes,
                                               self._st()))

    def replay_scatter(self, src, dst_rows, storage):
        assert storage.is_contiguous() and src.is_contiguous() and dst_rows.dtype == torch.int64
        row_bytes = storage[0].numel() * storage.element_size()
        self._ck(self.lib.b200rl_replay_scatter(_p(src), _p(dst_rows), _p(storage), dst_rows.numel(), row_bytes,
                                                self._st()))

    def gae(self, rewards, values, dones, next_value, gamma, lmbda, returns, advantages):
        _f32(rewards, values, dones, next_value, returns, advantages)
        T, E = rewards.shape[0], rewards[0].numel()
        self._ck(self.lib.b200rl_gae(_p(rewards), _p(values), _p(dones), _p(next_value), _p(returns), _p(advantages),
                                     T, E, gamma, lmbda, self._st()))

    EPI = {"none": 0, "relu": 1, "tanh": 2, "drelu": 3, "dtanh": 4}

    def bgemm(self, A, B, C, bias=None, aux=None, rsum=None, epi: str = "none", accumulate: bool = False):
        _f32(A, B, C, bias, aux, rsum)
        nets, M, N = C.shape
        K = A.shape[2]
        assert A.shape[1:] == (M, K) and B.shape[1:] == (K, N) and C.stride(2) == 1, (A.shape, B.shape, C.shape)

        def ns(t):
            return 0 if t is None or t.shape[0] == 1 else t.stride(0)

        if aux is not None:
            assert aux.shape == C.shape and aux.stride(2) == 1
        if bias is not None:
            assert bias.shape[1] == N and (N == 1 or bias.stride(1) == 1)
        if rsum is not None:
            assert rsum.shape == (nets, M) and (M == 1 or rsum.stride(1) == 1)
        self._ck(self.lib.b200rl_bgemm(_p(A), A.stride(1), A.stride(2), ns(A), _p(B), B.stride(1), B.stride(2), ns(B),
                                       _p(C), C.stride(1), ns(C), _p(bias), ns(bias), _p(aux),
                                       0 if aux is None else aux.stride(1), ns(aux), _p(rsum), ns(rsum), M, N, K, nets,
                                       self.EPI[epi], int(accumulate), self._st()))

    def sac_sample_fwd(self, head, eps, scale, abias, action, logp, tanh_out=None):
        _f32(head, eps, scale, abias, action, logp, tanh_out)
        B, A = eps.shape
        assert head.shape == (B, 2 * A) and head.is_contiguous() and eps.is_contiguous() and action.stride(1) == 1
        self._ck(self.lib.b200rl_sac_sample_fwd(_p(head), _p(eps), _p(scale), _p(abias), _p(action), action.stride(0),
                                                _p(logp), _p(tanh_out), B, A, self._st()))

    def sac_sample_bwd(self, head, eps, tanh_y, scale, dact, log_alpha, dhead):
        _f32(head, eps, tanh_y, scale, dact, log_alpha, dhead)
        nets, B, A = dact.shape
        assert dact.is_contiguous() and dhead.is_contiguous() and head.is_contiguous()
        self._ck(self.lib.b200rl_sac_sample_bwd(_p(head), _p(eps), _p(tanh_y), _p(scale), _p(dact), B * A, nets,
                                                _p(log_alpha), _p(dhead), B, A, self._st()))

    def sac_target(self, q_target, logp, rewards, terminated, log_alpha, gamma: float, y):
        _f32(q_target, logp, rewards, terminated, log_alpha, y)
        nets, B = q_target.shape
        assert q_target.is_contiguous()
        self._ck(self.lib.b200rl_sac_target(_p(q_target), B, nets, _p(logp), _p(rewards), _p(terminated), _p(log_alpha),
                                            gamma, _p(y), B, self._st()))

    def sac_critic_loss(self, q, y, dq, loss_out):
        _f32(q, y, dq, loss_out)
        nets, B = q.shape
        assert q.is_contiguous() and dq.is_contiguous()
        self._ck(self.lib.b200rl_sac_critic_loss(_p(q), B, nets, _p(y), _p(dq), _p(loss_out), B, self._st()))

    def sac_actor_loss(self, q, logp, log_alpha, target_entropy: float, dq, actor_loss, alpha_loss, dlog_alpha):
        _f32(q, logp, log_alpha, dq, actor_loss, alpha_loss, dlog_alpha)
        nets, B = q.shape
        assert q.is_contiguous() and dq.is_contiguous()
        self._ck(self.lib.b200rl_sac_actor_loss(_p(q), B, nets, _p(logp), _p(log_alpha), target_entropy, _p(dq),
                                                _p(actor_loss), _p(alpha_loss), _p(dlog_alpha), B, self._st()))

    def fill_normal(self, out, seed: int, stream_id: int, counter=None):
        _f32(out)
        self._ck(self.lib.b200rl_fill_normal(_p(out), out.numel(), seed, stream_id, _p(counter), self._st()))

    def droq_actor_loss(self, q, logp, log_alpha, target_entropy: float, dq, actor_loss, alpha_loss, dlog_alpha):
        _f32(q, logp, log_alpha, dq, actor_loss, alpha_loss, dlog_alpha)
        nets, B = q.shape
        assert q.is_contiguous() and dq.is_contiguous()
        self._ck(self.lib.b200rl_droq_actor_loss(_p(q), B, nets, _p(logp), _p(log_alpha), target_entropy, _p(dq),
                                                 _p(actor_loss), _p(alpha_loss), _p(dlog_alpha), B, self._st()))

    def dropout_mask(self, mask, p: float, seed: int, stream_id: int, counter=None):
        assert mask.dtype == torch.int32 and mask.is_cuda and mask.is_contiguous()
        self._ck(self.lib.b200rl_dropout_mask(_p(mask), mask.numel(), p, seed, stream_id, _p(counter), self._st()))

    def dropout_ln_relu_supported(self, H: int) -> bool:
        return bool(self.lib.b200rl_dropout_ln_relu_supported(H))

    @staticmethod
    def _dln_args(z, mask, gamma, stats):
        nets, B, H = z.shape
        assert z.is_contiguous() and stats.is_contiguous() and stats.shape == (nets, B, 2)
        assert gamma.shape == (nets, H) and (H == 1 or gamma.stride(1) == 1)
        if mask is not None:
            assert mask.dtype == torch.int32 and mask.is_contiguous() and mask.shape == (nets, B, (H + 31) // 32)
        return nets, B, H, (gamma.stride(0) if nets > 1 else H)

    def dropout_ln_relu_fwd(self, z, mask, p: float, gamma, beta, eps: float, y, stats):
        _f32(z, gamma, beta, y, stats)
        nets, B, H, sp = self._dln_args(z, mask, gamma, stats)
        assert y.shape == z.shape and y.is_contiguous() and beta.stride() == gamma.stride()
        self._ck(self.lib.b200rl_dropout_ln_relu_fwd(_p(z), _p(mask), p, _p(gamma), _p(beta), sp, eps, _p(y), _p(stats),
                                                     nets, B, H, self._st()))

    def dropout_ln_relu_bwd(self, dy, y, z, mask, p: float, stats, gamma, dz, dgamma=None, dbeta=None):
        _f32(dy, y, z, stats, gamma, dz, dgamma, dbeta)
        nets, B, H, sp = self._dln_args(z, mask, gamma, stats)
        for t in (dy, y, dz):
            assert t.shape == z.shape and t.is_contiguous()
        for t in (dgamma, dbeta):
            assert t is None or t.stride() == gamma.stride()
        self._ck(self.lib.b200rl_dropout_ln_relu_bwd(_p(dy), _p(y), _p(z), _p(mask), p, _p(stats), _p(gamma), sp,
                                                     _p(dz), _p(dgamma), _p(dbeta), nets, B, H, self._st()))

    def im2col(self, x, col, k: int, stride: int):
        _f32(x, col)
        B, H, W, C = x.shape
        assert x.is_contiguous() and col.is_contiguous()
        self._ck(self.lib.b200rl_im2col(_p(x), _p(col), B, H, W, C, k, stride, self._st()))

    def col2im(self, dcol, act, dx, k: int, stride: int):
        _f32(dcol, act, dx)
        B, H, W, C = dx.shape
        assert dx.is_contiguous() and dcol.is_contiguous() and (act is None or act.is_contiguous())
        self._ck(self.lib.b200rl_col2im(_p(dcol), _p(act), _p(dx), B, H, W, C, k, stride, self._st()))

    def ppo_loss(self, head, actions, old_logp, adv, values, old_values, returns, dhead, dvalues, losses, head_dims,
                 is_continuous: bool, clip_vloss: bool, normalize_adv: bool, clip_coef: float, vf_coef: float,
                 ent_coef: float):
        _f32(head, actions, old_logp, adv, values, old_values, returns, dhead, dvalues, losses)
        for t in (head, actions, dhead):
            assert t.is_contiguous()
        dims = (ctypes.c_int * len(head_dims))(*head_dims)
        self._ck(self.lib.b200rl_ppo_loss(_p(head), _p(actions), _p(old_logp), _p(adv), _p(values), _p(old_values),
                                          _p(returns), _p(dhead), _p(dvalues), _p(losses), head.shape[0], dims,
                                          len(head_dims), int(is_continuous), int(clip_vloss), int(normalize_adv),
                                          clip_coef, vf_coef, ent_coef, self._st()))

    def ppo_loss_masked(self, head, actions, old_logp, adv, values, old_values, returns, mask, dhead, dvalues, losses,
                        head_dims, is_continuous: bool, clip_vloss: bool, normalize_adv: bool, clip_coef: float,
                        vf_coef: float, ent_coef: float):
        _f32(head, actions, old_logp, adv, values, old_values, returns, mask, dhead, dvalues, losses)
        for t in (head, actions, dhead, mask):
            assert t.is_contiguous()
        dims = (ctypes.c_int * len(head_dims))(*head_dims)
        self._ck(self.lib.b200rl_ppo_loss_masked(_p(head), _p(actions), _p(old_logp), _p(adv), _p(values),
                                                 _p(old_values), _p(returns), _p(mask), _p(dhead), _p(dvalues),
                                                 _p(losses), head.shape[0], dims, len(head_dims), int(is_continuous),
                                                 int(clip_vloss), int(normalize_adv), clip_coef, vf_coef, ent_coef,
                                                 self._st()))

    def a2c_loss(self, head, actions, adv, values, returns, dhead, dvalues, losses, seg: int, head_dims,
                 is_continuous: int, normalize_adv: bool, reduce_sum: bool, vf_coef: float, ent_coef: float):
        _f32(head, actions, adv, values, returns, dhead, dvalues, losses)
        for t in (head, actions, adv, values, returns, dhead, dvalues, losses):
            assert t.is_contiguous()
        N = head.shape[0]
        assert losses.numel() == 3 * ((N + seg - 1) // seg)
        dims = (ctypes.c_int * len(head_dims))(*head_dims)
        self._ck(self.lib.b200rl_a2c_loss(_p(head), _p(actions), _p(adv), _p(values), _p(returns), _p(dhead),
                                          _p(dvalues), _p(losses), N, seg, dims, len(head_dims), int(is_continuous),
                                          int(normalize_adv), int(reduce_sum), vf_coef, ent_coef, self._st()))

    def lstm_seq_fwd(self, xw, W_hh, h0, c0, lengths, out, gates=None, cs=None, hT=None, cT=None):
        _f32(xw, W_hh, h0, c0, out, gates, cs, hT, cT)
        T, B, G = xw.shape
        H = G // 4
        assert lengths.dtype == torch.int32 and lengths.is_cuda and lengths.numel() == B
        for t in (xw, W_hh, h0, c0, lengths, out, gates, cs, hT, cT):
            assert t is None or t.is_contiguous()
        assert W_hh.shape == (G, H) and out.numel() == T * B * H and h0.numel() == B * H and c0.numel() == B * H
        self._ck(self.lib.b200rl_lstm_seq_fwd(_p(xw), _p(W_hh), _p(h0), _p(c0), _p(lengths), _p(out), _p(gates), _p(cs),
                                              _p(hT), _p(cT), T, B, H, self._st()))

    def lstm_seq_bwd(self, d_out, W_hh, gates, cs, c0, lengths, d_gates):
        _f32(d_out, W_hh, gates, cs, c0, d_gates)
        T, B, G = d_gates.shape
        H = G // 4
        assert lengths.dtype == torch.int32 and lengths.is_cuda and lengths.numel() == B
        for t in (d_out, W_hh, gates, cs, c0, lengths, d_gates):
            assert t.is_contiguous()
        self._ck(self.lib.b200rl_lstm_seq_bwd(_p(d_out), _p(W_hh), _p(gates), _p(cs), _p(c0), _p(lengths), _p(d_gates),
                                              T, B, H, self._st()))

    def transpose2d(self, X, Y):
        _f32(X, Y)
        rows, cols = X.shape
        self._ck(self.lib.b200rl_transpose2d(_p(X), _p(Y), rows, cols, _ld(X), _ld(Y), self._st()))

    def onehot_linear_supported(self, groups: int, classes: int, A: int, N: int) -> bool:
        return bool(self.lib.b200rl_onehot_linear_supported(groups, classes, A, N))

    def onehot_linear(self, z, act, WT, out, groups: int, classes: int):
        _f32(z, act, WT, out)
        M, A, N = z.shape[0], act.shape[1], WT.shape[1]
        assert WT.is_contiguous() and WT.shape[0] == groups * classes + A and out.shape == (M, N)
        self._ck(self.lib.b200rl_onehot_linear(_p(z), _p(act), _p(WT), _p(out), M, groups, classes, A, N, _ld(z),
                                               _ld(act), _ld(out), self._st()))

    def onehot_linear_ln_supported(self, WT, out, pre=None) -> bool:
        return bool(self.lib.b200rl_onehot_linear_ln_supported(_p(WT), None, None, _p(out), _p(pre), WT.shape[1],
                                                               _ld(out), _ld(pre)))

    def onehot_linear_ln(self, z, act, WT, gamma, beta, eps: float, out, groups: int, classes: int, pre=None):
        _f32(z, act, WT, gamma, beta, out, pre)
        M, A, N = z.shape[0], act.shape[1], WT.shape[1]
        assert WT.is_contiguous() and WT.shape[0] == groups * classes + A and out.shape == (M, N)
        self._ck(self.lib.b200rl_onehot_linear_ln(_p(z), _p(act), _p(WT), _p(gamma), _p(beta), eps, _p(pre), _ld(pre),
                                                  _p(out), M, groups, classes, A, N, _ld(z), _ld(act), _ld(out),
                                                  self._st()))

    def cont_action_fwd(self, head, eps, action, ent, min_std: float, max_std: float, init_std: float, clip: float):
        _f32(head, eps, action, ent)
        M, A = eps.shape
        assert head.shape == (M, 2 * A) and head.is_contiguous() and eps.is_contiguous()
        self._ck(self.lib.b200rl_cont_action_fwd(_p(head), _p(eps), _p(action), _ld(action), _p(ent), M, A, min_std,
                                                 max_std, init_std, clip, self._st()))

    def cont_action_bwd(self, head, eps, d_action, discount, dhead, min_std: float, max_std: float, init_std: float,
                        clip: float, ent_scale: float):
        _f32(head, eps, d_action, discount, dhead)
        M, A = eps.shape
        assert head.is_contiguous() and eps.is_contiguous() and dhead.is_contiguous() and discount.numel() >= M
        self._ck(self.lib.b200rl_cont_action_bwd(_p(head), _p(eps), _p(d_action), _ld(d_action), _p(discount),
                                                 _p(dhead), M, A, min_std, max_std, init_std, clip, ent_scale,
                                                 self._st()))

    def lambda_returns_bwd(self, cont_logit, discount, moments, lam, val, ent, gamma, lmbda, ent_coef, scale, d_val,
                           d_rew, rows):
        _f32(cont_logit, discount, moments, lam, val, ent, d_val, d_rew, rows)
        H, N = lam.shape
        self._ck(self.lib.b200rl_lambda_returns_bwd(_p(cont_logit), _p(discount), _p(moments), _p(lam), _p(val), _p(ent),
                                                    _p(d_val), _p(d_rew), _p(rows), H, N, gamma, lmbda, ent_coef, scale,
                                                    self._st()))

    def twohot_mean_bwd(self, logits, d_mean, low: float, high: float, d_logits):
        _f32(logits, d_mean, d_logits)
        M, nb = logits.shape
        self._ck(self.lib.b200rl_twohot_mean_bwd(_p(logits), _p(d_mean), _p(d_logits), M, nb, _ld(logits), _ld(d_logits),
                                                 low, high, self._st()))

    def ppo_act(self, head, noise, actions, logp, head_dims, is_continuous: bool, greedy: bool):
        _f32(head, noise, actions, logp)
        assert head.is_contiguous() and actions.is_contiguous() and (noise is None or noise.is_contiguous())
        dims = (ctypes.c_int * len(head_dims))(*head_dims)
        self._ck(self.lib.b200rl_ppo_act(_p(head), _p(noise), _p(actions), _p(logp), head.shape[0], dims,
                                         len(head_dims), int(is_continuous), int(greedy), self._st()))
```

Measured before the change: 58.07.

## Pre-split weights into TF32 hi/lo planes outside the tensor-core GEMM and conv kernels

Adds a PRESPLIT variant of the warp-specialized TMA GEMM kernel in which the weight operand is loaded as ready-made TF32 hi and lo planes, so the in-kernel split warps and their barrier are skipped. Weight planes are produced by separate split, transposed-split and conv pack kernels, and the conv paths and large-M GEMMs route through the presplit path. Pipeline stage counts are now derived from the shared-memory budget, so the presplit variant can run deeper stages. The cost is an extra split kernel launch and extra memory traffic for weights on every call, plus TMA loads of two B planes instead of one.

```diff
diff --git a/include/b200rl.h b/include/b200rl.h
--- a/include/b200rl.h
+++ b/include/b200rl.h
@@ -20,11 +20,24 @@
                              int transB);
 int b200rl_gemm_tc(const float* A, const float* B, float* C, const float* bias, int M, int N, int K, int lda, int ldb,
                    int ldc, int transA, int transB, int accumulate, cudaStream_t stream);
+int b200rl_tf32_split(const float* X, float* Xhi, float* Xlo, long long n, cudaStream_t stream);
+int b200rl_tf32_split_t(const float* W, float* Thi, float* Tlo, int rows, int cols, long long ldw, long long ldt,
+                        cudaStream_t stream);
+int b200rl_gemm_tc_presplit_supported(const float* A, const float* Bhi, const float* Blo, int M, int N, int K, int lda,
+                                      int ldb);
+int b200rl_gemm_tc_presplit(const float* A, const float* Bhi, const float* Blo, float* C, const float* bias, int M, int N,
+                            int K, int lda, int ldb, int ldc, int accumulate, cudaStream_t stream);
 int b200rl_gemm_ln_supported(const float* A, const float* W, int M, int N, int K, int lda, int ldw, int mode);
 int b200rl_gemm_ln(const float* A, const float* W, int M, int N, int K, int lda, int ldw, const float* gamma,
                    const float* beta, float eps, int act, float* pre, long long ldpre, float* out, long long ldout,
                    int mode, const float* h_prev, long long ldh, float* h_out, long long ldho, float* h_out2,
                    long long ldho2, cudaStream_t stream);
+int b200rl_gemm_ln_presplit_supported(const float* A, const float* Whi, const float* Wlo, int M, int N, int K, int lda,
+                                      int ldw, int mode);
+int b200rl_gemm_ln_presplit(const float* A, const float* Whi, const float* Wlo, int M, int N, int K, int lda, int ldw,
+                            const float* gamma, const float* beta, float eps, int act, float* pre, long long ldpre,
+                            float* out, long long ldout, int mode, const float* h_prev, long long ldh, float* h_out,
+                            long long ldho, float* h_out2, long long ldho2, cudaStream_t stream);
 int b200rl_ln_act_fwd(const float* X, const float* gamma, const float* beta, float* Y, long long M, int C,
                       long long ldx, long long ldy, float eps, int act, cudaStream_t stream);
 int b200rl_ln_act_bwd(const float* X, const float* gamma, const float* beta, const float* dY, float* dX, float* dgamma,
@@ -56,6 +69,11 @@
                         cudaStream_t stream);
 int b200rl_conv_up_tc(const float* small_, const float* Wpacked, float* big, const float* bias, int NB, int h, int w,
                       int Cs, int Cb, cudaStream_t stream);
+int b200rl_conv_pack_split(const float* W, float* Whi, float* Wlo, int mode_up, int Cs, int Cb, cudaStream_t stream);
+int b200rl_conv_down_tc_presplit(const float* big, const float* Whi, const float* Wlo, float* small_, int NB, int h, int w,
+                                 int Cs, int Cb, cudaStream_t stream);
+int b200rl_conv_up_tc_presplit(const float* small_, const float* Whi, const float* Wlo, float* big, const float* bias,
+                               int NB, int h, int w, int Cs, int Cb, cudaStream_t stream);
 
 int b200rl_gru_gate_fwd(const float* G, const float* Hin, float* Hout, long long M, int R, long long ldg,
                         long long ldhi, long long ldho, cudaStream_t stream);
diff --git a/sheeprl_b200/csrc/gemm_tc.cu b/sheeprl_b200/csrc/gemm_tc.cu
--- a/sheeprl_b200/csrc/gemm_tc.cu
+++ b/sheeprl_b200/csrc/gemm_tc.cu
@@ -13,7 +13,10 @@
 constexpr int NSPLIT_THREADS = 96;
 constexpr int NCONS_WARPS = 8;
 constexpr int PRODUCER_REGS = 56, CONSUMER_REGS = 224;
-template <int BN> constexpr int stages_for() { return BN == 128 ? 3 : 5; }
+template <int PASSES, bool PRESPLIT> __host__ __device__ constexpr int b_buffers() { return PRESPLIT ? (PASSES == 3 ? 2 : 1) : 3; }
+template <int BN, int PASSES, bool PRESPLIT> constexpr int stages_for() {
+  return (227 * 1024 - 1024 - 256) / ((BM + b_buffers<PASSES, PRESPLIT>() * BN) * BK * (int)sizeof(float));
+}
 
 __device__ __forceinline__ uint32_t smem_u32(const void* p) { return (uint32_t)__cvta_generic_to_shared(p); }
 
@@ -117,14 +120,24 @@
   return (uint32_t)((r >> 5) * 4096 + k * 128 + (((((r & 31) >> 2) ^ k) & 7) << 4) + (r & 3) * 4);
 }
 
-template <int BN>
-struct Smem {
-  static constexpr int STAGES = stages_for<BN>();
+template <int BN, int PASSES, bool PRESPLIT>
+struct Smem;
+template <int BN, int PASSES>
+struct Smem<BN, PASSES, false> {
+  static constexpr int STAGES = stages_for<BN, PASSES, false>();
   float a[STAGES][BM * BK];
   float b[STAGES][BN * BK];
   float b_hi[STAGES][BN * BK];
   float b_lo[STAGES][BN * BK];
   uint64_t full[STAGES], split[STAGES], empty[STAGES];
+};
+template <int BN, int PASSES>
+struct Smem<BN, PASSES, true> {
+  static constexpr int STAGES = stages_for<BN, PASSES, true>();
+  float a[STAGES][BM * BK];
+  float b_hi[STAGES][BN * BK];
+  float b_lo[PASSES == 3 ? STAGES : 1][PASSES == 3 ? BN * BK : 256];
+  uint64_t full[STAGES], empty[STAGES];
 };
 
 constexpr int CH = 4;
@@ -150,13 +163,15 @@
   int wg;
 };
 
-template <int BN, int PASSES>
+template <int BN, int PASSES, bool PRESPLIT>
 __global__ void __launch_bounds__(NTHREADS, 1)
-gemm_tc_kernel(const __grid_constant__ CUtensorMap mapA, const __grid_constant__ CUtensorMap mapB, float* __restrict__ C,
-               const float* __restrict__ bias, int M, int N, int K, int ldc, int accumulate, const TileGeo geo) {
-  constexpr int STAGES = Smem<BN>::STAGES;
+gemm_tc_kernel(const __grid_constant__ CUtensorMap mapA, const __grid_constant__ CUtensorMap mapB,
+               const __grid_constant__ CUtensorMap mapBlo, float* __restrict__ C, const float* __restrict__ bias, int M,
+               int N, int K, int ldc, int accumulate, const TileGeo geo) {
+  using S = Smem<BN, PASSES, PRESPLIT>;
+  constexpr int STAGES = S::STAGES;
   extern __shared__ __align__(1024) unsigned char smem_raw[];
-  Smem<BN>& s = *reinterpret_cast<Smem<BN>*>(smem_raw + ((1024u - (smem_u32(smem_raw) & 1023u)) & 1023u));
+  S& s = *reinterpret_cast<S*>(smem_raw + ((1024u - (smem_u32(smem_raw) & 1023u)) & 1023u));
   const int warp = threadIdx.x >> 5, lane = threadIdx.x & 31;
   const int mtiles = geo.mtiles * geo.ntiles, tstride = gridDim.y;
   auto tile_mn = [&](int id, int& tm, int& tn) {
@@ -182,7 +197,7 @@
   if (threadIdx.x == 0) {
     for (int i = 0; i < STAGES; ++i) {
       mbar_init(&s.full[i], 1);
-      mbar_init(&s.split[i], NSPLIT_THREADS / 32);
+      if constexpr (!PRESPLIT) mbar_init(&s.split[i], NSPLIT_THREADS / 32);
       mbar_init(&s.empty[i], NCONS_WARPS);
     }
     asm volatile("fence.mbarrier_init.release.cluster;" ::: "memory");
@@ -193,6 +208,15 @@
     asm volatile("setmaxnreg.dec.sync.aligned.u32 %0;" ::"n"(PRODUCER_REGS));
     if (warp == 0) {
       const bool leader = elect_one();
+      constexpr uint32_t STAGE_TX = (uint32_t)((BM + (PRESPLIT ? b_buffers<PASSES, true>() : 1) * BN) * BK * sizeof(float));
+      auto load_b_kmajor = [&](int st, int k, int n) {
+        if constexpr (PRESPLIT) {
+          tma_load_2d(s.b_hi[st], &mapB, &s.full[st], k, n);
+          if (PASSES == 3) tma_load_2d(s.b_lo[st], &mapBlo, &s.full[st], k, n);
+        } else {
+          tma_load_2d(s.b[st], &mapB, &s.full[st], k, n);
+        }
+      };
       int it = 0;
       for (int tile = blockIdx.y; tile < mtiles; tile += tstride) {
         int tm, tn;
@@ -204,7 +228,7 @@
           const int st = it % STAGES;
           if (it >= STAGES) mbar_wait(&s.empty[st], ((it / STAGES) - 1) & 1);
           if (leader) {
-            mbar_expect_tx(&s.full[st], (uint32_t)((BM + BN) * BK * sizeof(float)));
+            mbar_expect_tx(&s.full[st], STAGE_TX);
             if (geo.mode == MODE_GEMM) {
               const int k0 = (kb_base + kb) * BK;
               if (geo.wg) {
@@ -216,8 +240,8 @@
               } else if (!geo.a_mn) tma_load_2d(s.a[st], &mapA, &s.full[st], k0, m0);
               else
                 for (int j = 0; j < BM / 32; ++j) tma_load_2d(s.a[st] + j * 1024, &mapA, &s.full[st], m0 + 32 * j, k0);
-              if (!geo.b_mn) tma_load_2d(s.b[st], &mapB, &s.full[st], k0, n0);
-              else
+              if (PRESPLIT || !geo.b_mn) load_b_kmajor(st, k0, n0);
+              else if constexpr (!PRESPLIT)
                 for (int j = 0; j < BN / 32; ++j) tma_load_2d(s.b[st] + j * 1024, &mapB, &s.full[st], n0 + 32 * j, k0);
             } else {
               const int tap = kb / geo.chunks, ch = (kb - tap * geo.chunks) * BK;
@@ -226,13 +250,13 @@
               else if (geo.mode == MODE_UP4) { x = tx0 + (tap % 3) - 1;     y = ty0 + (tap / 3) - 1; }
               else                           { x = tx0 + px - (tap & 1);    y = ty0 + py - (tap >> 1); }
               tma_load_4d(s.a[st], &mapA, &s.full[st], ch, x, y, tn0);
-              tma_load_2d(s.b[st], &mapB, &s.full[st], kb * BK, n0 + (geo.mode == MODE_UP ? (int)blockIdx.z * geo.Cout : 0));
+              load_b_kmajor(st, kb * BK, n0 + (geo.mode == MODE_UP ? (int)blockIdx.z * geo.Cout : 0));
             }
           }
           __syncwarp();
         }
       }
-    } else {
+    } else if constexpr (!PRESPLIT) {
       const int t = threadIdx.x - 32;
       int ntl = 0;
       for (int tile = blockIdx.y; tile < mtiles; tile += tstride) ++ntl;
@@ -294,7 +318,7 @@
         const int st = it % STAGES;
         const uint32_t ph = (it / STAGES) & 1;
         mbar_wait(&s.full[st], ph);
-        mbar_wait(&s.split[st], ph);
+        if constexpr (!PRESPLIT) mbar_wait(&s.split[st], ph);
         const char* araw = reinterpret_cast<const char*>(s.a[st]);
         uint32_t ahi[4][4], alo[4][4];
 #pragma unroll
@@ -507,15 +531,50 @@
   return gy < (unsigned)tiles ? gy : (unsigned)tiles;
 }
 
-__global__ void conv_pack_down_kernel(const float* __restrict__ W, float* __restrict__ P, int Cs, int Cb) {
+__device__ __forceinline__ float tf32_hi(float x) { return __uint_as_float(__float_as_uint(x) & 0xffffe000u); }
+__device__ __forceinline__ void store_split(float* P, float* L, long long i, float v) {
+  if (L) { const float h = tf32_hi(v); P[i] = h; L[i] = v - h; }
+  else P[i] = v;
+}
+
+__global__ void tf32_split_kernel(const float* __restrict__ X, float* __restrict__ H, float* __restrict__ L, long long n) {
+  const long long i = ((long long)blockIdx.x * blockDim.x + threadIdx.x) * 4;
+  if (i + 4 <= n && !((reinterpret_cast<uintptr_t>(X) | reinterpret_cast<uintptr_t>(H) | reinterpret_cast<uintptr_t>(L)) & 15)) {
+    const float4 v = *reinterpret_cast<const float4*>(X + i);
+    const float4 h = make_float4(tf32_hi(v.x), tf32_hi(v.y), tf32_hi(v.z), tf32_hi(v.w));
+    *reinterpret_cast<float4*>(H + i) = h;
+    *reinterpret_cast<float4*>(L + i) = make_float4(v.x - h.x, v.y - h.y, v.z - h.z, v.w - h.w);
+  } else {
+    for (long long j = i; j < i + 4 && j < n; ++j) store_split(H, L, j, X[j]);
+  }
+}
+
+__global__ void tf32_split_t_kernel(const float* __restrict__ W, float* __restrict__ H, float* __restrict__ L, int rows,
+                                    int cols, long long ldw, long long ldt) {
+  __shared__ float t[32][33];
+  const int c0 = blockIdx.x * 32, r0 = blockIdx.y * 32;
+  for (int j = threadIdx.y; j < 32; j += blockDim.y) {
+    const int r = r0 + j, c = c0 + threadIdx.x;
+    t[j][threadIdx.x] = (r < rows && c < cols) ? W[(long long)r * ldw + c] : 0.f;
+  }
+  __syncthreads();
+  for (int j = threadIdx.y; j < 32; j += blockDim.y) {
+    const int c = c0 + j, r = r0 + threadIdx.x;
+    if (c < cols && r < ldt) store_split(H, L, (long long)c * ldt + r, t[threadIdx.x][j]);
+  }
+}
+
+__global__ void conv_pack_down_kernel(const float* __restrict__ W, float* __restrict__ P, float* __restrict__ L, int Cs,
+                                      int Cb) {
   const long long idx = (long long)blockIdx.x * blockDim.x + threadIdx.x;
   if (idx >= (long long)Cs * Cb * 16) return;
   const int cb = (int)(idx % Cb);
   const int tap = (int)((idx / Cb) % 16);
   const int cs = (int)(idx / ((long long)Cb * 16));
-  P[idx] = W[((long long)cs * Cb + cb) * 16 + tap];
-}
-__global__ void conv_pack_up_kernel(const float* __restrict__ W, float* __restrict__ P, int Cs, int Cb) {
+  store_split(P, L, idx, W[((long long)cs * Cb + cb) * 16 + tap]);
+}
+__global__ void conv_pack_up_kernel(const float* __restrict__ W, float* __restrict__ P, float* __restrict__ L, int Cs,
+                                    int Cb) {
   const long long idx = (long long)blockIdx.x * blockDim.x + threadIdx.x;
   if (idx >= (long long)Cs * Cb * 16) return;
   const int cs = (int)(idx % Cs);
@@ -524,10 +583,11 @@
   const int par = (int)(idx / ((long long)Cs * 4 * Cb));
   const int py = par >> 1, px = par & 1;
   const int ky = (1 - py) + 2 * (t >> 1), kx = (1 - px) + 2 * (t & 1);
-  P[idx] = W[((long long)cs * Cb + cb) * 16 + ky * 4 + kx];
-}
-
-__global__ void conv_pack_up4_kernel(const float* __restrict__ W, float* __restrict__ P, int Cs, int Cb) {
+  store_split(P, L, idx, W[((long long)cs * Cb + cb) * 16 + ky * 4 + kx]);
+}
+
+__global__ void conv_pack_up4_kernel(const float* __restrict__ W, float* __restrict__ P, float* __restrict__ L, int Cs,
+                                     int Cb) {
   const long long idx = (long long)blockIdx.x * blockDim.x + threadIdx.x;
   if (idx >= 36LL * Cs * Cb) return;
   const int cs = (int)(idx % Cs);
@@ -538,7 +598,7 @@
   const int j = py - dy, i = px - dx;
   float v = 0.f;
   if (j >= 0 && j <= 1 && i >= 0 && i <= 1) v = W[((long long)cs * Cb + cb) * 16 + ((1 - py) + 2 * j) * 4 + (1 - px) + 2 * i];
-  P[idx] = v;
+  store_split(P, L, idx, v);
 }
 static bool conv_up_merged(int Cb) { return Cb == 32; }
 
@@ -605,25 +665,32 @@
   }
 }
 
-#define LAUNCH_GEMM_TC(BN_, PASSES_, grid_, st_, ...)                                                                \
+#define LAUNCH_GEMM_TC(BN_, PASSES_, PRE_, grid_, st_, ...)                                                          \
   do {                                                                                                               \
-    const size_t smem__ = sizeof(Smem<BN_>) + 1024;                                                                  \
-    RL_CUDA(cudaFuncSetAttribute(gemm_tc_kernel<BN_, PASSES_>, cudaFuncAttributeMaxDynamicSharedMemorySize, (int)smem__)); \
-    gemm_tc_kernel<BN_, PASSES_><<<grid_, NTHREADS, smem__, st_>>>(__VA_ARGS__);                                      \
+    static_assert(sizeof(Smem<BN_, PASSES_, PRE_>) + 1024 <= 227 * 1024, "operand stages exceed shared memory");     \
+    const size_t smem__ = sizeof(Smem<BN_, PASSES_, PRE_>) + 1024;                                                   \
+    RL_CUDA(cudaFuncSetAttribute(gemm_tc_kernel<BN_, PASSES_, PRE_>, cudaFuncAttributeMaxDynamicSharedMemorySize,     \
+                                 (int)smem__));                                                                      \
+    gemm_tc_kernel<BN_, PASSES_, PRE_><<<grid_, NTHREADS, smem__, st_>>>(__VA_ARGS__);                                \
   } while (0)
-#define DISPATCH_GEMM_TC(BN_val, passes_val, grid_, st_, ...)                                  \
+#define DISPATCH_GEMM_TC_PRE(BN_val, passes_val, PRE_, grid_, st_, ...)                        \
   do {                                                                                          \
     if ((BN_val) == 64) {                                                                       \
-      if ((passes_val) == 3) LAUNCH_GEMM_TC(64, 3, grid_, st_, __VA_ARGS__);                    \
-      else LAUNCH_GEMM_TC(64, 1, grid_, st_, __VA_ARGS__);                                      \
+      if ((passes_val) == 3) LAUNCH_GEMM_TC(64, 3, PRE_, grid_, st_, __VA_ARGS__);              \
+      else LAUNCH_GEMM_TC(64, 1, PRE_, grid_, st_, __VA_ARGS__);                                \
     } else {                                                                                    \
-      if ((passes_val) == 3) LAUNCH_GEMM_TC(128, 3, grid_, st_, __VA_ARGS__);                   \
-      else LAUNCH_GEMM_TC(128, 1, grid_, st_, __VA_ARGS__);                                     \
+      if ((passes_val) == 3) LAUNCH_GEMM_TC(128, 3, PRE_, grid_, st_, __VA_ARGS__);             \
+      else LAUNCH_GEMM_TC(128, 1, PRE_, grid_, st_, __VA_ARGS__);                               \
     }                                                                                           \
   } while (0)
-
-int launch_conv(int mode, const float* img, const float* Wp, float* out, const float* bias, int NB, int h, int w, int Cin,
-                int Cout, cudaStream_t st) {
+#define DISPATCH_GEMM_TC(BN_val, passes_val, presplit_, grid_, st_, ma_, mb_, mb2_, ...)                    \
+  do {                                                                                                       \
+    if (presplit_) DISPATCH_GEMM_TC_PRE(BN_val, passes_val, true, grid_, st_, ma_, mb_, mb2_, __VA_ARGS__);  \
+    else DISPATCH_GEMM_TC_PRE(BN_val, passes_val, false, grid_, st_, ma_, mb_, mb_, __VA_ARGS__);           \
+  } while (0)
+
+int launch_conv(int mode, const float* img, const float* Wp, const float* Wlo, float* out, const float* bias, int NB, int h,
+                int w, int Cin, int Cout, cudaStream_t st) {
   TileGeo g = {};
   g.mode = mode; g.h = h; g.w = w; g.NB = NB; g.chunks = Cin / BK; g.Cout = Cout; g.ksplits = 1;
   g.passes = g_passes;
@@ -638,13 +705,15 @@
   const int BN = (mode == MODE_UP4) ? 128 : ((Cout <= 64) ? 64 : 128);
   const int brows = (mode == MODE_UP || mode == MODE_UP4) ? 4 * Cout : Cout;
   if (int rc = get_map(Wp, brows, K, K, BN, &mb)) return rc;
+  CUtensorMap mb2 = mb;
+  if (Wlo && g.passes == 3) { if (int rc = get_map(Wlo, brows, K, K, BN, &mb2)) return rc; }
   const int mtiles = g.tiles_x * g.tiles_y * (NB / g.bn);
   g.mtiles = mtiles;
   g.ntiles = (mode == MODE_UP4) ? 1 : (Cout + BN - 1) / BN;
   dim3 grid(1, 1, mode == MODE_UP ? 4 : 1);
   grid.y = persistent_grid_y(mtiles * g.ntiles, grid.z);
   const int M = NB * h * w;
-  DISPATCH_GEMM_TC(BN, g.passes, grid, st, ma, mb, out, bias, M, Cout, K, Cout, 0, g);
+  DISPATCH_GEMM_TC(BN, g.passes, Wlo != nullptr, grid, st, ma, mb, mb2, out, bias, M, Cout, K, Cout, 0, g);
   RL_CHECK_LAUNCH();
   return B200RL_OK;
 }
@@ -668,26 +737,65 @@
   if (Cin % BK != 0 || Cout < 16 || Cout % 4 != 0) return 0;
   return 1;
 }
+namespace {
+int conv_pack_impl(const float* W, float* P, float* L, int mode_up, int Cs, int Cb, cudaStream_t st) {
+  const long long n = (long long)Cs * Cb * 16;
+  if (mode_up && conv_up_merged(Cb)) conv_pack_up4_kernel<<<ceil_div(36LL * Cs * Cb, 256), 256, 0, st>>>(W, P, L, Cs, Cb);
+  else if (mode_up) conv_pack_up_kernel<<<ceil_div(n, 256), 256, 0, st>>>(W, P, L, Cs, Cb);
+  else conv_pack_down_kernel<<<ceil_div(n, 256), 256, 0, st>>>(W, P, L, Cs, Cb);
+  RL_CHECK_LAUNCH();
+  return B200RL_OK;
+}
+}
 extern "C" int b200rl_conv_pack(const float* W, float* Wpacked, int mode_up, int Cs, int Cb, cudaStream_t st) {
   RL_CHECK_ARG(W && Wpacked, "null pointer");
-  const long long n = (long long)Cs * Cb * 16;
-  if (mode_up && conv_up_merged(Cb)) conv_pack_up4_kernel<<<ceil_div(36LL * Cs * Cb, 256), 256, 0, st>>>(W, Wpacked, Cs, Cb);
-  else if (mode_up) conv_pack_up_kernel<<<ceil_div(n, 256), 256, 0, st>>>(W, Wpacked, Cs, Cb);
-  else conv_pack_down_kernel<<<ceil_div(n, 256), 256, 0, st>>>(W, Wpacked, Cs, Cb);
-  RL_CHECK_LAUNCH();
-  return B200RL_OK;
+  return conv_pack_impl(W, Wpacked, nullptr, mode_up, Cs, Cb, st);
+}
+extern "C" int b200rl_conv_pack_split(const float* W, float* Whi, float* Wlo, int mode_up, int Cs, int Cb, cudaStream_t st) {
+  RL_CHECK_ARG(W && Whi && Wlo, "null pointer");
+  return conv_pack_impl(W, Whi, Wlo, mode_up, Cs, Cb, st);
 }
 extern "C" int b200rl_conv_down_tc(const float* big, const float* Wpacked, float* small_, int NB, int h, int w, int Cs,
                                    int Cb, cudaStream_t st) {
   RL_CHECK_ARG(big && Wpacked && small_, "null pointer");
   RL_CHECK_ARG(b200rl_conv_tc_supported(0, NB, h, w, Cs, Cb), "shape not eligible for the tensor-core conv path");
-  return launch_conv(MODE_DOWN, big, Wpacked, small_, nullptr, NB, h, w, Cb, Cs, st);
+  return launch_conv(MODE_DOWN, big, Wpacked, nullptr, small_, nullptr, NB, h, w, Cb, Cs, st);
 }
 extern "C" int b200rl_conv_up_tc(const float* small_, const float* Wpacked, float* big, const float* bias, int NB, int h,
                                  int w, int Cs, int Cb, cudaStream_t st) {
   RL_CHECK_ARG(big && Wpacked && small_, "null pointer");
   RL_CHECK_ARG(b200rl_conv_tc_supported(1, NB, h, w, Cs, Cb), "shape not eligible for the tensor-core conv path");
-  return launch_conv(MODE_UP, small_, Wpacked, big, bias, NB, h, w, Cs, Cb, st);
+  return launch_conv(MODE_UP, small_, Wpacked, nullptr, big, bias, NB, h, w, Cs, Cb, st);
+}
+extern "C" int b200rl_conv_down_tc_presplit(const float* big, const float* Whi, const float* Wlo, float* small_, int NB,
+                                            int h, int w, int Cs, int Cb, cudaStream_t st) {
+  RL_CHECK_ARG(big && Whi && Wlo && small_, "null pointer");
+  RL_CHECK_ARG(b200rl_conv_tc_supported(0, NB, h, w, Cs, Cb), "shape not eligible for the tensor-core conv path");
+  return launch_conv(MODE_DOWN, big, Whi, Wlo, small_, nullptr, NB, h, w, Cb, Cs, st);
+}
+extern "C" int b200rl_conv_up_tc_presplit(const float* small_, const float* Whi, const float* Wlo, float* big,
+                                          const float* bias, int NB, int h, int w, int Cs, int Cb, cudaStream_t st) {
+  RL_CHECK_ARG(big && Whi && Wlo && small_, "null pointer");
+  RL_CHECK_ARG(b200rl_conv_tc_supported(1, NB, h, w, Cs, Cb), "shape not eligible for the tensor-core conv path");
+  return launch_conv(MODE_UP, small_, Whi, Wlo, big, bias, NB, h, w, Cs, Cb, st);
+}
+
+extern "C" int b200rl_tf32_split(const float* X, float* Xhi, float* Xlo, long long n, cudaStream_t st) {
+  RL_CHECK_ARG(X && Xhi && Xlo, "null pointer");
+  RL_CHECK_ARG(n >= 0, "negative length");
+  if (n == 0) return B200RL_OK;
+  tf32_split_kernel<<<ceil_div((n + 3) / 4, 256), 256, 0, st>>>(X, Xhi, Xlo, n);
+  RL_CHECK_LAUNCH();
+  return B200RL_OK;
+}
+extern "C" int b200rl_tf32_split_t(const float* W, float* Thi, float* Tlo, int rows, int cols, long long ldw, long long ldt,
+                                   cudaStream_t st) {
+  RL_CHECK_ARG(W && Thi && Tlo, "null pointer");
+  RL_CHECK_ARG(rows > 0 && cols > 0 && ldw >= cols && ldt >= rows, "bad transposed-split geometry");
+  dim3 grid(ceil_div(cols, 32), ceil_div(ldt, 32));
+  tf32_split_t_kernel<<<grid, dim3(32, 8), 0, st>>>(W, Thi, Tlo, rows, cols, ldw, ldt);
+  RL_CHECK_LAUNCH();
+  return B200RL_OK;
 }
 
 extern "C" int b200rl_gemm_tc_supported(const float* A, const float* B, int M, int N, int K, int lda, int ldb,
@@ -702,16 +810,19 @@
 namespace {
 struct FusedTail { float* part; int ks, mpad, ldw; };
 
-int gemm_tc_impl(const float* A, const float* B, float* C, const float* bias, int M, int N, int K, int lda,
-                 int ldb, int ldc, int transA, int transB, int accumulate, cudaStream_t st, FusedTail* fused) {
+int gemm_tc_impl(const float* A, const float* B, const float* Blo, float* C, const float* bias, int M, int N, int K,
+                 int lda, int ldb, int ldc, int transA, int transB, int accumulate, cudaStream_t st, FusedTail* fused) {
   RL_CHECK_ARG(A && B && (C || fused), "null pointer");
   RL_CHECK_ARG(b200rl_gemm_tc_supported(A, B, M, N, K, lda, ldb, transA, transB), "shape not eligible for the tensor-core path");
+  RL_CHECK_ARG(!Blo || (transB && !(reinterpret_cast<uintptr_t>(Blo) & 15)), "pre-split B must be 16-byte aligned [N][K] planes");
   const int BN = (N <= 64) ? 64 : 128;
-  CUtensorMap ma, mb;
+  CUtensorMap ma, mb, mb2;
   if (!transA) { if (int rc = get_map(A, M, K, lda, BM, &ma)) return rc; }
   else         { if (int rc = get_map(A, K, M, lda, 32, &ma)) return rc; }
   if (transB)  { if (int rc = get_map(B, N, K, ldb, BN, &mb)) return rc; }
   else         { if (int rc = get_map(B, K, N, ldb, 32, &mb)) return rc; }
+  mb2 = mb;
+  if (Blo && g_passes == 3) { if (int rc = get_map(Blo, N, K, ldb, BN, &mb2)) return rc; }
   dim3 grid((N + BN - 1) / BN, (M + BM - 1) / BM);
   TileGeo g = {};
   g.mode = MODE_GEMM;
@@ -743,7 +854,7 @@
   g.ntiles = (int)grid.x;
   grid.x = 1;
   grid.y = persistent_grid_y(g.mtiles * g.ntiles, grid.z);
-  DISPATCH_GEMM_TC(BN, g.passes, grid, st, ma, mb, C, bias, M, N, K, ldc, accumulate, g);
+  DISPATCH_GEMM_TC(BN, g.passes, Blo != nullptr, grid, st, ma, mb, mb2, C, bias, M, N, K, ldc, accumulate, g);
   RL_CHECK_LAUNCH();
   if (g.ksplits > 1 && !fused) {
     splitk_reduce_kernel<<<ceil_div((long long)M * ((N + 3) / 4), 256), 256, 0, st>>>(g.part, C, bias, M, N, ldc, g.ksplits, g.mpad,
@@ -834,7 +945,17 @@
 
 extern "C" int b200rl_gemm_tc(const float* A, const float* B, float* C, const float* bias, int M, int N, int K, int lda,
                               int ldb, int ldc, int transA, int transB, int accumulate, cudaStream_t st) {
-  return gemm_tc_impl(A, B, C, bias, M, N, K, lda, ldb, ldc, transA, transB, accumulate, st, nullptr);
+  return gemm_tc_impl(A, B, nullptr, C, bias, M, N, K, lda, ldb, ldc, transA, transB, accumulate, st, nullptr);
+}
+
+extern "C" int b200rl_gemm_tc_presplit_supported(const float* A, const float* Bhi, const float* Blo, int M, int N, int K,
+                                                 int lda, int ldb) {
+  return b200rl_gemm_tc_supported(A, Bhi, M, N, K, lda, ldb, 0, 1) && !(reinterpret_cast<uintptr_t>(Blo) & 15);
+}
+extern "C" int b200rl_gemm_tc_presplit(const float* A, const float* Bhi, const float* Blo, float* C, const float* bias, int M,
+                                       int N, int K, int lda, int ldb, int ldc, int accumulate, cudaStream_t st) {
+  RL_CHECK_ARG(Blo, "null pointer");
+  return gemm_tc_impl(A, Bhi, Blo, C, bias, M, N, K, lda, ldb, ldc, 0, 1, accumulate, st, nullptr);
 }
 
 extern "C" int b200rl_gemm_ln_supported(const float* A, const float* B, int M, int N, int K, int lda, int ldb, int mode) {
@@ -844,10 +965,11 @@
   return 1;
 }
 
-extern "C" int b200rl_gemm_ln(const float* A, const float* W, int M, int N, int K, int lda, int ldw_, const float* gamma,
-                              const float* beta, float eps, int act, float* pre, long long ldpre, float* out, long long ldout,
-                              int mode, const float* h_prev, long long ldh, float* h_out, long long ldho, float* h_out2,
-                              long long ldho2, cudaStream_t st) {
+namespace {
+int gemm_ln_impl(const float* A, const float* W, const float* Wlo, int M, int N, int K, int lda, int ldw_, const float* gamma,
+                 const float* beta, float eps, int act, float* pre, long long ldpre, float* out, long long ldout, int mode,
+                 const float* h_prev, long long ldh, float* h_out, long long ldho, float* h_out2, long long ldho2,
+                 cudaStream_t st) {
   RL_CHECK_ARG(A && W && gamma && beta, "null pointer");
   RL_CHECK_ARG(b200rl_gemm_ln_supported(A, W, M, N, K, lda, ldw_, mode), "shape not eligible for the fused product + LayerNorm");
   RL_CHECK_ARG(mode == 0 ? out != nullptr : (h_prev && h_out), "missing output");
@@ -857,7 +979,7 @@
                    ((ldpre | ldout | ldh | ldho | ldho2) & 3) == 0,
                "fused product + LayerNorm needs 16-byte aligned rows");
   FusedTail ft;
-  if (int rc = gemm_tc_impl(A, W, nullptr, nullptr, M, N, K, lda, ldw_, N, 0, 1, 0, st, &ft)) return rc;
+  if (int rc = gemm_tc_impl(A, W, Wlo, nullptr, nullptr, M, N, K, lda, ldw_, N, 0, 1, 0, st, &ft)) return rc;
   const int blocks = ceil_div((long long)M * 32, 256);
 #define LAUNCH_SPLITK_LN(NV_)                                                                                              \
   splitk_ln_kernel<NV_><<<blocks, 256, 0, st>>>(ft.part, ft.ks, ft.mpad, ft.ldw, M, N, gamma, beta, eps, act, pre, ldpre, out, \
@@ -873,6 +995,28 @@
 #undef LAUNCH_SPLITK_LN
   RL_CHECK_LAUNCH();
   return B200RL_OK;
+}
+}
+
+extern "C" int b200rl_gemm_ln(const float* A, const float* W, int M, int N, int K, int lda, int ldw_, const float* gamma,
+                              const float* beta, float eps, int act, float* pre, long long ldpre, float* out, long long ldout,
+                              int mode, const float* h_prev, long long ldh, float* h_out, long long ldho, float* h_out2,
+                              long long ldho2, cudaStream_t st) {
+  return gemm_ln_impl(A, W, nullptr, M, N, K, lda, ldw_, gamma, beta, eps, act, pre, ldpre, out, ldout, mode, h_prev, ldh,
+                      h_out, ldho, h_out2, ldho2, st);
+}
+extern "C" int b200rl_gemm_ln_presplit_supported(const float* A, const float* Whi, const float* Wlo, int M, int N, int K,
+                                                 int lda, int ldw, int mode) {
+  return b200rl_gemm_ln_supported(A, Whi, M, N, K, lda, ldw, mode) && !(reinterpret_cast<uintptr_t>(Wlo) & 15);
+}
+extern "C" int b200rl_gemm_ln_presplit(const float* A, const float* Whi, const float* Wlo, int M, int N, int K, int lda,
+                                       int ldw, const float* gamma, const float* beta, float eps, int act, float* pre,
+                                       long long ldpre, float* out, long long ldout, int mode, const float* h_prev,
+                                       long long ldh, float* h_out, long long ldho, float* h_out2, long long ldho2,
+                                       cudaStream_t st) {
+  RL_CHECK_ARG(Wlo, "null pointer");
+  return gemm_ln_impl(A, Whi, Wlo, M, N, K, lda, ldw, gamma, beta, eps, act, pre, ldpre, out, ldout, mode, h_prev, ldh,
+                      h_out, ldho, h_out2, ldho2, st);
 }
 
 extern "C" int b200rl_conv_wgrad_mn_supported(int NB, int h, int w, int Cs, int Cb) {
@@ -913,7 +1057,7 @@
   }
   grid.x = 1;
   grid.y = (unsigned)(g.mtiles * g.ntiles);
-  DISPATCH_GEMM_TC(BN, g.passes, grid, st, ma, mb, G, nullptr, M, N, P, N, 0, g);
+  DISPATCH_GEMM_TC(BN, g.passes, false, grid, st, ma, mb, mb, G, nullptr, M, N, P, N, 0, g);
   RL_CHECK_LAUNCH();
   if (g.ksplits > 1) {
     splitk_reduce_kernel<<<ceil_div((long long)M * ((N + 3) / 4), 256), 256, 0, st>>>(g.part, G, nullptr, M, N, N, g.ksplits, g.mpad,
diff --git a/sheeprl_b200/lib.py b/sheeprl_b200/lib.py
--- a/sheeprl_b200/lib.py
+++ b/sheeprl_b200/lib.py
@@ -12,6 +12,8 @@
 HEADER_PATH = os.path.join(os.path.dirname(_HERE), "include", "b200rl.h")
 
 _lib = None
+
+PRESPLIT_MIN_ROWS = 4096
 
 
 class B200RLError(RuntimeError):
@@ -163,8 +165,25 @@
         assert (A.shape[1] if transA else A.shape[0]) == M, (A.shape, C.shape, transA)
         assert (B.shape[0] if transB else B.shape[1]) == N and (B.shape[1] if transB else B.shape[0]) == K, \
             (A.shape, B.shape, C.shape, transA, transB)
+        if (not transA and M >= PRESPLIT_MIN_ROWS and self.use_tc
+                and self.lib.b200rl_gemm_tc_supported(_p(A), _p(B), M, N, K, _ld(A), _ld(B), 0, int(transB))):
+            hi, lo, ld = self._planes(B, transB, N, K)
+            self._ck(self.lib.b200rl_gemm_tc_presplit(_p(A), _p(hi), _p(lo), _p(C), _p(bias), M, N, K, _ld(A), ld, _ld(C),
+                                                      int(accumulate), self._st()))
+            return
         self._ck(self.lib.b200rl_gemm_f32(_p(A), _p(B), _p(C), _p(bias), M, N, K, _ld(A), _ld(B), _ld(C), int(transA),
                                           int(transB), int(accumulate), self._st()))
+
+    def _planes(self, B, transB: bool, N: int, K: int):
+        ldb = _ld(B)
+        ld = ldb if transB else (K + 3) // 4 * 4
+        buf = self._scratch("b_planes", 2 * N * ld)
+        hi, lo = buf[:N * ld], buf[N * ld:2 * N * ld]
+        if transB:
+            self._ck(self.lib.b200rl_tf32_split(_p(B), _p(hi), _p(lo), (N - 1) * ldb + K, self._st()))
+        else:
+            self._ck(self.lib.b200rl_tf32_split_t(_p(B), _p(hi), _p(lo), K, N, ldb, ld, self._st()))
+        return hi, lo, ld
 
     def gemm_ln_supported(self, A, W, mode: int = 0) -> bool:
         M, K = A.shape
@@ -229,8 +248,9 @@
         Cb = big.shape[-1]
         assert tuple(big.shape) == (NB, 2 * h, 2 * w, Cb) and tuple(W.shape) == (Cs, Cb, 4, 4)
         if self.use_tc and self.lib.b200rl_conv_tc_supported(0, NB, h, w, Cs, Cb):
-            Wp = self._packed(W, 0, Cs, Cb)
-            self._ck(self.lib.b200rl_conv_down_tc(_p(big), _p(Wp), _p(small), NB, h, w, Cs, Cb, self._st()))
+            hi, lo = self._packed(W, 0, Cs, Cb)
+            self._ck(self.lib.b200rl_conv_down_tc_presplit(_p(big), _p(hi), _p(lo), _p(small), NB, h, w, Cs, Cb,
+                                                           self._st()))
             return
         self._ck(self.lib.b200rl_conv_down(_p(big), _p(W), _p(small), NB, h, w, Cs, Cb, self._st()))
 
@@ -238,11 +258,11 @@
         key = (W.data_ptr(), mode_up)
         buf = self._pack_bufs.get(key)
         need = self.lib.b200rl_conv_pack_floats(mode_up, Cs, Cb)
-        if buf is None or buf.numel() != need:
-            buf = torch.empty(need, dtype=torch.float32, device=W.device)
+        if buf is None or buf.shape != (2, need):
+            buf = torch.empty(2, need, dtype=torch.float32, device=W.device)
             self._pack_bufs[key] = buf
-        self._ck(self.lib.b200rl_conv_pack(_p(W), _p(buf), mode_up, Cs, Cb, self._st()))
-        return buf
+        self._ck(self.lib.b200rl_conv_pack_split(_p(W), _p(buf[0]), _p(buf[1]), mode_up, Cs, Cb, self._st()))
+        return buf[0], buf[1]
 
     def conv_up(self, small, W, big, bias=None):
         _f32(big, W, small, bias)
@@ -251,8 +271,9 @@
         Cb = big.shape[-1]
         assert tuple(big.shape) == (NB, 2 * h, 2 * w, Cb) and tuple(W.shape) == (Cs, Cb, 4, 4)
         if self.use_tc and self.lib.b200rl_conv_tc_supported(1, NB, h, w, Cs, Cb):
-            Wp = self._packed(W, 1, Cs, Cb)
-            self._ck(self.lib.b200rl_conv_up_tc(_p(small), _p(Wp), _p(big), _p(bias), NB, h, w, Cs, Cb, self._st()))
+            hi, lo = self._packed(W, 1, Cs, Cb)
+            self._ck(self.lib.b200rl_conv_up_tc_presplit(_p(small), _p(hi), _p(lo), _p(big), _p(bias), NB, h, w, Cs, Cb,
+                                                         self._st()))
             return
         self._ck(self.lib.b200rl_conv_up(_p(small), _p(W), _p(big), _p(bias), NB, h, w, Cs, Cb, self._st()))
 
```

Result: faster. 60.10 (median of 6 runs) (+3.5%).
